# AssafSinger94/dino-tracker

Measured on NVIDIA B200. Metric: query-points/sec (854x476, T=50), higher is better.
Workload: dtype f32

## Files before the change

dino_tracker_b200/_lib.py:

```python
import ctypes
import os
from ctypes import POINTER, Structure, c_char_p, c_float, c_int, c_size_t, c_ulonglong, c_void_p

import torch

from . import build as _build

_LIB = None


class Geom(Structure):
    _fields_ = [("H", c_int), ("W", c_int), ("patch", c_int), ("stride", c_int), ("radius", c_int),
                ("h", c_int), ("w", c_int)]


class HeadWeights(Structure):
    _fields_ = [("w1", c_float * 9 * 16), ("b1", c_float * 16), ("w2", c_float * 9 * 16), ("b2", c_float)]


class Features(Structure):
    _fields_ = [("tpc", c_void_p), ("norms", c_void_p), ("hi", c_void_p), ("lo", c_void_p), ("T", c_int), ("C", c_int)]


class VitConfig(Structure):
    _fields_ = [("depth", c_int), ("dim", c_int), ("heads", c_int), ("tap_layer", c_int), ("patch", c_int), ("stride", c_int),
                ("attn_materialized", c_int), ("gemm_f16", c_int), ("gemm_pair", c_int)]


class VitWeights(Structure):
    _fields_ = [("patch_w", c_void_p), ("patch_b", c_void_p), ("cls_pos", c_void_p), ("pos", c_void_p),
                ("blocks", POINTER(c_void_p))]


class DinotrkError(RuntimeError):
    pass


_P = c_void_p
SIGNATURES = {
    "dinotrk_version": (c_int, []),
    "dinotrk_last_error": (c_char_p, []),
    "dinotrk_launch_count": (c_ulonglong, []),
    "dinotrk_make_geom": (c_int, [c_int, c_int, c_int, c_int, c_int, POINTER(Geom)]),
    "dinotrk_pack_features": (c_int, [_P, _P, _P, c_int, c_int, c_int, _P]),
    "dinotrk_unpack_features": (c_int, [_P, _P, c_int, c_int, c_int, _P]),
    "dinotrk_token_norms": (c_int, [_P, _P, c_int, c_int, c_int, _P]),
    "dinotrk_sample_descriptors": (c_int, [_P, c_int, c_int, POINTER(Geom), _P, c_int, _P, c_int, c_int, _P, _P, _P]),
    "dinotrk_split_fp16": (c_int, [_P, _P, _P, c_size_t, _P]),
    "dinotrk_corr_track_workspace_bytes": (c_size_t, [c_int, c_int, c_int, POINTER(Geom)]),
    "dinotrk_corr_track": (c_int, [POINTER(Features), POINTER(Geom), POINTER(HeadWeights), _P, _P, _P, _P, _P, _P,
                                   c_int, c_int, c_int, _P, _P, c_int, c_int, _P, c_size_t, _P]),
    "dinotrk_corr_maps_workspace_bytes": (c_size_t, [c_int, c_int, c_int]),
    "dinotrk_map_stride": (c_int, [POINTER(Geom)]),
    "dinotrk_corr_maps": (c_int, [POINTER(Features), POINTER(Geom), _P, _P, _P, _P, _P, _P, c_int, c_int, c_int,
                                  _P, _P, c_size_t, _P]),
    "dinotrk_head": (c_int, [_P, c_int, POINTER(Geom), POINTER(HeadWeights), _P, _P, c_int, c_int, _P, _P, _P]),
    "dinotrk_sample_backward": (c_int, [c_int, c_int, POINTER(Geom), _P, c_int, _P, c_int, c_int, _P, _P, _P]),
    "dinotrk_track_backward_workspace_bytes": (c_size_t, [c_int, c_int, POINTER(Geom)]),
    "dinotrk_track_backward": (c_int, [POINTER(Features), POINTER(Geom), POINTER(HeadWeights), _P, _P, c_int, _P, _P, _P, _P, _P,
                                       _P, c_int, _P, _P, _P, c_size_t, _P]),
    "dinotrk_infer_workspace_bytes": (c_size_t, [c_int, c_int, POINTER(Geom), c_int, c_int]),
    "dinotrk_infer_set_overlap": (c_int, [c_int]),
    "dinotrk_infer_set_path": (c_int, [c_int]),
    "dinotrk_infer_last_stats": (c_int, [POINTER(ctypes.c_longlong), c_int]),
    "dinotrk_infer_max_chunks": (c_size_t, [c_int, c_int, c_int]),
    "dinotrk_infer_plan": (c_int, [c_int, c_int, c_int, _P, c_int, _P, _P, c_int, _P]),
    "dinotrk_infer": (c_int, [POINTER(Features), POINTER(Geom), POINTER(HeadWeights), _P, c_int, c_float, c_float,
                              c_int, c_int, c_int, c_int, _P, _P, _P, _P, _P, c_size_t, _P]),
    "dinotrk_traj_cos_sims": (c_int, [_P, c_int, c_int, POINTER(Geom), _P, _P, c_int, _P, _P, c_size_t, _P]),
    "dinotrk_delta_workspace_bytes": (c_size_t, [c_int, c_int, c_int, POINTER(c_int)]),
    "dinotrk_delta_refine": (c_int, [_P, c_int, c_int, c_int, POINTER(c_int), POINTER(c_void_p), POINTER(c_void_p), _P,
                                     _P, _P, c_int, c_int, _P, _P, _P, c_size_t, _P]),
    "dinotrk_vit_workspace_bytes": (c_size_t, [POINTER(VitConfig), POINTER(Geom), c_int]),
    "dinotrk_vit_attention": (c_int, [_P, _P, _P, c_int, c_int, c_int, c_int, _P, _P]),
    "dinotrk_vit_forward": (c_int, [_P, c_int, POINTER(Geom), POINTER(VitConfig), POINTER(VitWeights), _P, _P, c_size_t, _P]),
    "dinotrk_best_buddies_workspace_bytes": (c_size_t, [c_int, c_int]),
    "dinotrk_best_buddies_pairs": (c_int, [POINTER(Features), POINTER(Geom), _P, _P, c_int, _P, _P, _P, c_size_t, _P]),
    "dinotrk_bb_mutual": (c_int, [_P, _P, c_int, c_int, _P, _P]),
    "dinotrk_bb_nms": (c_int, [_P, c_int, POINTER(Geom), c_float, c_float, c_int, _P, _P, _P]),
    "dinotrk_profile_classes": (c_int, []),
    "dinotrk_profile_class_name": (c_char_p, [c_int]),
    "dinotrk_profile_enable": (None, [c_int]),
    "dinotrk_profile_collect": (c_int, [POINTER(ctypes.c_double), POINTER(c_ulonglong), c_int]),
    "dinotrk_delta_refine_allgather": (c_int, [_P, c_int, c_int, c_int, POINTER(c_int), POINTER(c_void_p), POINTER(c_void_p), _P,
                                               _P, _P, c_int, c_int, _P, _P, _P, c_size_t, POINTER(c_void_p), c_int, c_size_t, _P]),
    "dinotrk_delta_refine_tc": (c_int, [_P, c_int, c_int, c_int, POINTER(c_int), POINTER(c_void_p), POINTER(c_void_p),
                                        POINTER(c_void_p), _P, _P, _P, c_int, c_int, _P, _P, _P, c_size_t, POINTER(c_void_p),
                                        c_int, c_size_t, _P]),
    "dinotrk_peer_alloc": (c_int, [c_size_t, POINTER(c_void_p), ctypes.c_char_p]),
    "dinotrk_peer_open": (c_int, [ctypes.c_char_p, POINTER(c_void_p)]),
    "dinotrk_peer_close": (c_int, [_P]),
    "dinotrk_peer_free": (c_int, [_P]),
    "dinotrk_occlusion": (c_int, [_P, _P, _P, c_int, c_int, c_float, c_float, _P, _P]),
}


def lib_path():
    return _build.LIB_PATH


def load(build_if_missing=True):
    global _LIB
    if _LIB is not None:
        return _LIB
    path = lib_path()
    if not os.path.exists(path):
        if not build_if_missing:
            raise DinotrkError(f"{path} is missing: run `python -c 'import __graft_entry__ as g; g.build()'`")
        _build.build()
    lib = ctypes.CDLL(path)
    for name, (res, args) in SIGNATURES.items():
        fn = getattr(lib, name)
        fn.restype = res
        fn.argtypes = args
    if lib.dinotrk_version() < 100:
        raise DinotrkError("libdinotrk.so is older than the Python binding")
    _LIB = lib
    return lib


def check(rc, what="dinotrk"):
    if rc != 0:
        raise DinotrkError(f"{what} failed ({rc}): {load().dinotrk_last_error().decode()}")


def ptr(t):
    if t is None:
        return None
    assert t.is_cuda and t.is_contiguous(), "device pointers must come from contiguous CUDA tensors"
    return c_void_p(t.data_ptr())


def stream_ptr(device=None):
    return c_void_p(torch.cuda.current_stream(device).cuda_stream)


def on_device(fn):
    import functools

    @functools.wraps(fn)
    def wrapped(self, *a, **kw):
        with torch.cuda.device(self._dev):
            return fn(self, *a, **kw)
    return wrapped


def require_cuda(device):
    if not torch.cuda.is_available():
        raise DinotrkError("dino_tracker_b200 needs a CUDA device (sm_100a); there is no CPU fallback")
    dev = torch.device(device)
    if dev.type != "cuda":
        raise DinotrkError(f"dino_tracker_b200 runs on CUDA only, got device={device!r}")
    return dev


def make_features(tpc, norms, hi=None, lo=None):
    f = Features()
    f.tpc, f.norms = tpc.data_ptr(), norms.data_ptr()
    f.hi = hi.data_ptr() if hi is not None else None
    f.lo = lo.data_ptr() if lo is not None else None
    f.T, f.C = tpc.shape[0], tpc.shape[2]
    f._keep = (tpc, norms, hi, lo)
    return f


def make_geom(H, W, patch=14, stride=7, radius=35):
    g = Geom()
    check(load().dinotrk_make_geom(H, W, patch, stride, radius, ctypes.byref(g)), "make_geom")
    return g


def profile_enable(on=True):
    load().dinotrk_profile_enable(1 if on else 0)


def profile_collect():
    lib = load()
    n = lib.dinotrk_profile_classes()
    ms = (ctypes.c_double * n)()
    cnt = (c_ulonglong * n)()
    check(lib.dinotrk_profile_collect(ms, cnt, n), "profile_collect")
    return {lib.dinotrk_profile_class_name(i).decode(): (ms[i], int(cnt[i])) for i in range(n) if cnt[i]}


def infer_stats():
    a = (ctypes.c_longlong * 5)()
    check(load().dinotrk_infer_last_stats(a, 5), "infer_last_stats")
    return {"anchor_maps": int(a[0]), "exact_window": int(a[1]), "full_map": int(a[2]), "pipeline": "exact-window" if a[3] else "full-map",
            "full_map_by_certificate": int(a[4])}


def launch_count():
    return int(load().dinotrk_launch_count())
```

dino_tracker_b200/csrc/inference.cu:

```cuda
#include <algorithm>
#include <vector>

#include "common.cuh"
#include "corr.cuh"
#include "sample.cuh"
#include "xwin.cuh"

namespace dtk {

constexpr int TC2_BM_ROWS = 256;

__global__ void sample_query_kernel(const float* __restrict__ tpc, int T, int C, int P, int h, int w, PointAffine pa,
                                    const float* __restrict__ qp, float* __restrict__ desc, float* __restrict__ dnorm) {
  int n = blockIdx.x;
  float x = __fadd_rn(__fmul_rn(pa.aw, qp[n * 3 + 0]), pa.bw);
  float y = __fadd_rn(__fmul_rn(pa.ah, qp[n * 3 + 1]), pa.bh);
  int tq = (int)qp[n * 3 + 2];
  tq = min(max(tq, 0), T - 1);
  TriCorners c = tri_setup(x, y, 0.f, 2, h, w);
  sample_point(tpc, C, P, c, tq, -1, desc + (size_t)n * C, dnorm + n);
}

__global__ void index_traj_kernel(const int* __restrict__ grp_frame, const int* __restrict__ grp_row0,
                                  const int* __restrict__ grp_map0, int n_groups, int n_maps, int T,
                                  int* __restrict__ out_index, float* __restrict__ traj) {
  int j = blockIdx.x * blockDim.x + threadIdx.x;
  if (j >= n_maps) return;
  int lo = 0, hi = n_groups - 1;
  while (lo < hi) {
    int mid = (lo + hi + 1) >> 1;
    if (grp_map0[mid] <= j) lo = mid; else hi = mid - 1;
  }
  int n = grp_row0[lo] + (j - grp_map0[lo]);
  int t = grp_frame[lo];
  out_index[j] = n * T + t;
  traj[((size_t)n * T + t) * 3 + 2] = (float)t;
}

__global__ void traj_cos_kernel(const float* __restrict__ tpc, int T, int C, int P, int h, int w, PointAffine pa,
                                const float* __restrict__ traj, const float* __restrict__ qp,
                                float* __restrict__ cos_out) {
  extern __shared__ __align__(16) float sm[];
  __shared__ float nrm[2];
  __shared__ float red[SAMPLE_THREADS / 32];
  const int n = blockIdx.y, i = blockIdx.x;
  int tq = (int)qp[n * 3 + 2];
  tq = min(max(tq, 0), T - 1);
  for (int which = 0; which < 2; ++which) {
    const float* pt = traj + ((size_t)n * T + (which == 0 ? tq : i)) * 3;
    float x = __fadd_rn(__fmul_rn(pa.aw, pt[0]), pa.bw);
    float y = __fadd_rn(__fmul_rn(pa.ah, pt[1]), pa.bh);
    TriCorners c = tri_setup(x, y, pt[2], T, h, w);
    sample_point(tpc, C, P, c, c.z0, c.z1, sm + which * C, nrm + which);
    __syncthreads();
  }
  const float nq = fmaxf(nrm[0], 1e-8f), ni = fmaxf(nrm[1], 1e-8f);
  float acc = 0.f;
  for (int c = threadIdx.x; c < C; c += SAMPLE_THREADS) acc = fmaf(__fdiv_rn(sm[c], nq), __fdiv_rn(sm[C + c], ni), acc);
  acc = warp_sum(acc);
  if ((threadIdx.x & 31) == 0) red[threadIdx.x >> 5] = acc;
  __syncthreads();
  if (threadIdx.x == 0) {
    float s = 0.f;
    for (int k = 0; k < SAMPLE_THREADS / 32; ++k) s += red[k];
    cos_out[(size_t)n * T + i] = s;
  }
}

__global__ void anchor_lists_kernel(const float* __restrict__ cos_sims, int N, int T, float th,
                                    int* __restrict__ cnt, int* __restrict__ qlist) {
  const int a = blockIdx.x;
  __shared__ int base;
  __shared__ int wcount[32];
  if (threadIdx.x == 0) base = 0;
  __syncthreads();
  const int lane = threadIdx.x & 31, warp = threadIdx.x >> 5, nw = blockDim.x >> 5;
  for (int n0 = 0; n0 < N; n0 += blockDim.x) {
    int n = n0 + threadIdx.x;
    bool v = n < N && cos_sims[(size_t)n * T + a] >= th;
    unsigned bal = __ballot_sync(0xffffffffu, v);
    if (lane == 0) wcount[warp] = __popc(bal);
    __syncthreads();
    int off = base;
    for (int k = 0; k < warp; ++k) off += wcount[k];
    if (v) qlist[(size_t)a * N + off + __popc(bal & ((1u << lane) - 1))] = n;
    __syncthreads();
    if (threadIdx.x == 0) {
      int tot = 0;
      for (int k = 0; k < nw; ++k) tot += wcount[k];
      base += tot;
    }
    __syncthreads();
  }
  if (threadIdx.x == 0) cnt[a] = base;
}

__global__ void sample_anchor_kernel(const float* __restrict__ tpc, int T, int C, int P, int h, int w, PointAffine pa,
                                     const float* __restrict__ traj, const int* __restrict__ qlist, int N,
                                     const int* __restrict__ grp_frame, const int* __restrict__ grp_map0,
                                     const int* __restrict__ grp_item0, int n_groups, int frame_batch,
                                     float* __restrict__ desc, float* __restrict__ dnorm, int* __restrict__ out_index,
                                     __half* __restrict__ desc_hi, __half* __restrict__ desc_lo) {
  const int j = blockIdx.x;
  int lo = 0, hi = n_groups - 1;
  while (lo < hi) {
    int mid = (lo + hi + 1) >> 1;
    if (grp_map0[mid] <= j) lo = mid; else hi = mid - 1;
  }
  const int a = grp_frame[lo];
  const int u = grp_item0[lo] + (j - grp_map0[lo]);
  const int slot = u / T, i = u - slot * T;
  const int n = qlist[(size_t)a * N + slot];
  const int i0 = (i / frame_batch) * frame_batch, e = min(i0 + frame_batch, T);
  const int Nset = e - i0 + 1;
  const float* pt = traj + ((size_t)n * T + i) * 3;
  float x = __fadd_rn(__fmul_rn(pa.aw, pt[0]), pa.bw);
  float y = __fadd_rn(__fmul_rn(pa.ah, pt[1]), pa.bh);
  TriCorners c = tri_setup(x, y, (float)(i - i0 + 1), Nset, h, w);
  int f0 = c.z0 == 0 ? a : i0 + c.z0 - 1;
  int f1 = c.z1 < 0 ? -1 : (c.z1 == 0 ? a : i0 + c.z1 - 1);
  sample_point(tpc, C, P, c, f0, f1, desc + (size_t)j * C, dnorm + j, desc_hi ? desc_hi + (size_t)j * C : nullptr,
               desc_lo ? desc_lo + (size_t)j * C : nullptr);
  if (threadIdx.x == 0) out_index[j] = (n * T + a) * T + i;
}

__global__ void sample_unique_kernel(const float* __restrict__ tpc, int T, int C, int P, int h, int w, PointAffine pa,
                                     const float* __restrict__ traj, int frame_batch, __half* __restrict__ u_hi,
                                     __half* __restrict__ u_lo, float* __restrict__ u_norm, int* __restrict__ u_flag) {
  const int u = blockIdx.x;
  const int i = u % T;
  const int i0 = (i / frame_batch) * frame_batch, e = min(i0 + frame_batch, T);
  const float* pt = traj + (size_t)u * 3;
  float x = __fadd_rn(__fmul_rn(pa.aw, pt[0]), pa.bw);
  float y = __fadd_rn(__fmul_rn(pa.ah, pt[1]), pa.bh);
  TriCorners c = tri_setup(x, y, (float)(i - i0 + 1), e - i0 + 1, h, w);
  bool slot0 = false;
#pragma unroll
  for (int k = 0; k < 4; ++k) slot0 = slot0 || (c.z0 == 0 && c.tok[k] >= 0 && c.wxy[k][0] != 0.f);
  if (threadIdx.x == 0) u_flag[u] = slot0 ? 1 : 0;
  if (slot0) return;
  const int f0 = i0 + c.z0 - 1;
  const int f1 = c.z1 < 0 ? -1 : i0 + c.z1 - 1;
  sample_point(tpc, C, P, c, f0, f1, nullptr, u_norm + u, u_hi + (size_t)u * C, u_lo + (size_t)u * C);
}

__global__ void gather_anchor_kernel(const float* __restrict__ tpc, int T, int C, int P, int h, int w, PointAffine pa,
                                     const float* __restrict__ traj, const int* __restrict__ qlist, int N,
                                     const int* __restrict__ grp_frame, const int* __restrict__ grp_map0,
                                     const int* __restrict__ grp_item0, int n_groups, int frame_batch,
                                     const __half* __restrict__ u_hi, const __half* __restrict__ u_lo,
                                     const float* __restrict__ u_norm, const int* __restrict__ u_flag,
                                     float* __restrict__ dnorm, int* __restrict__ out_index, __half* __restrict__ desc_hi,
                                     __half* __restrict__ desc_lo) {
  const int j = blockIdx.x;
  int lo = 0, hi = n_groups - 1;
  while (lo < hi) {
    int mid = (lo + hi + 1) >> 1;
    if (grp_map0[mid] <= j) lo = mid; else hi = mid - 1;
  }
  const int a = grp_frame[lo];
  const int uu = grp_item0[lo] + (j - grp_map0[lo]);
  const int slot = uu / T, i = uu - slot * T;
  const int n = qlist[(size_t)a * N + slot];
  const size_t u = (size_t)n * T + i;
  if (threadIdx.x == 0) out_index[j] = (n * T + a) * T + i;
  if (!u_flag[u]) {
    const uint4* sh = reinterpret_cast<const uint4*>(u_hi + u * C);
    const uint4* sl = reinterpret_cast<const uint4*>(u_lo + u * C);
    uint4* dh = reinterpret_cast<uint4*>(desc_hi + (size_t)j * C);
    uint4* dl = reinterpret_cast<uint4*>(desc_lo + (size_t)j * C);
    for (int k = threadIdx.x; k < C / 8; k += blockDim.x) { dh[k] = __ldg(sh + k); dl[k] = __ldg(sl + k); }
    if (threadIdx.x == 0) dnorm[j] = u_norm[u];
    return;
  }
  const int i0 = (i / frame_batch) * frame_batch, e = min(i0 + frame_batch, T);
  const float* pt = traj + u * 3;
  float x = __fadd_rn(__fmul_rn(pa.aw, pt[0]), pa.bw);
  float y = __fadd_rn(__fmul_rn(pa.ah, pt[1]), pa.bh);
  TriCorners c = tri_setup(x, y, (float)(i - i0 + 1), e - i0 + 1, h, w);
  int f0 = c.z0 == 0 ? a : i0 + c.z0 - 1;
  int f1 = c.z1 < 0 ? -1 : (c.z1 == 0 ? a : i0 + c.z1 - 1);
  sample_point(tpc, C, P, c, f0, f1, nullptr, dnorm + j, desc_hi + (size_t)j * C, desc_lo + (size_t)j * C);
}

constexpr int OCC_THREADS = 256;
__global__ void occlusion_kernel(const float* __restrict__ traj, const float* __restrict__ cos_sims,
                                 const float* __restrict__ anchors, int T, float anchor_th, float cos_th,
                                 uint8_t* __restrict__ occ) {
  extern __shared__ float sm[];
  float* med = sm;
  int* alist = reinterpret_cast<int*>(sm + T);
  float* ax = sm + 2 * T;
  float* ay = sm + 3 * T;
  const int lane = threadIdx.x & 31, warp = threadIdx.x >> 5, nw = OCC_THREADS / 32;
  float* col = sm + 4 * T + warp * T;
  __shared__ int M;
  __shared__ float th_s;
  const int n = blockIdx.x;
  if (threadIdx.x == 0) {
    int m = 0;
    for (int a = 0; a < T; ++a)
      if (cos_sims[(size_t)n * T + a] >= anchor_th) {
        alist[m] = a;
        ax[m] = traj[((size_t)n * T + a) * 3 + 0];
        ay[m] = traj[((size_t)n * T + a) * 3 + 1];
        ++m;
      }
    M = m;
  }
  __syncthreads();
  const int m = M, want = (m - 1) / 2;
  for (int i = warp; i < T; i += nw) {
    for (int p = lane; p < m; p += 32) {
      const float* g = anchors + (((size_t)n * T + alist[p]) * T + i) * 2;
      float dx = __fsub_rn(g[0], ax[p]), dy = __fsub_rn(g[1], ay[p]);
      col[p] = sqrtf(__fadd_rn(__fmul_rn(dx, dx), __fmul_rn(dy, dy)));
    }
    __syncwarp();
    for (int p = lane; p < m; p += 32) {
      const float dp = col[p];
      int rank = 0;
      for (int q = 0; q < m; ++q) {
        float dq = col[q];
        rank += (dq < dp) || (dq == dp && q < p);
      }
      if (rank == want) med[i] = dp;
    }
    __syncwarp();
  }
  __syncthreads();
  if (threadIdx.x == 0) {
    float th = -INFINITY;
    for (int p = 0; p < m; ++p) th = fmaxf(th, med[alist[p]]);
    th_s = th;
  }
  __syncthreads();
  for (int i = threadIdx.x; i < T; i += blockDim.x)
    occ[(size_t)n * T + i] = (m > 0 && (med[i] > th_s || cos_sims[(size_t)n * T + i] < cos_th)) ? 1 : 0;
}

struct GroupBuf {
  std::vector<int> v;
  int cap, n;
  explicit GroupBuf(int c) : v((size_t)5 * c), cap(c), n(0) {}
  void clear() { n = 0; }
  void push(int frame, int row0, int m, int map0, int item0) {
    v[n] = frame; v[cap + n] = row0; v[2 * cap + n] = m; v[3 * cap + n] = map0; v[4 * cap + n] = item0; ++n;
  }
};

struct ChunkMeta { int used, maxm, n_groups; bool no_thin; };
static void plan_chunks(int kind, int T, int N, const int* cnt, int ch_all, int gcap, std::vector<ChunkMeta>& metas,
                        std::vector<int>& plan_host, int align = 1, int first_cap = 0) {
  int ch = ch_all;
  metas.clear(); plan_host.clear();
  GroupBuf gb(gcap);
  auto commit_chunk = [&](int used, int maxm) {
    bool no_thin = true;
    for (int k = 0; k < gb.n; ++k) no_thin = no_thin && gb.v[2 * gb.cap + k] > STREAM_MAX_M;
    metas.push_back(ChunkMeta{used, maxm, gb.n, no_thin});
    plan_host.insert(plan_host.end(), gb.v.begin(), gb.v.end());
  };
  if (kind == 0) {
    int t = 0, row = 0;
    while (t < T) {
      gb.clear();
      int used = 0, maxm = 0;
      while (t < T && used < ch && gb.n < gcap) {
        int m = N - row;
        if (m > ch - used) m = ch - used;
        gb.push(t, row, m, used, 0);
        used += m; row += m;
        if (m > maxm) maxm = m;
        if (row == N) { row = 0; ++t; }
      }
      commit_chunk(used, maxm);
    }
  } else {
    int a = 0;
    long long item = 0;
    while (a < T) {
      gb.clear();
      int used = 0, maxm = 0;
      ch = (metas.empty() && first_cap > 0 && first_cap < ch_all) ? first_cap : ch_all;
      while (a < T && used < ch && gb.n < gcap) {
        long long tot = (long long)cnt[a] * T;
        long long m = tot - item;
        if (m > ch - used) {
          m = (long long)((ch - used) / align) * align;
          if (m == 0 && used > 0) break;
          if (m == 0) m = align;
        }
        if (m > 0) {
          gb.push(a, used, (int)m, used, (int)item);
          used += (int)m; item += m;
          if ((int)m > maxm) maxm = (int)m;
        }
        if (item >= tot) { item = 0; ++a; }
      }
      if (used == 0) break;
      commit_chunk(used, maxm);
    }
  }
}

struct CellPlan {
  std::vector<int> v;
  std::vector<size_t> first;
  std::vector<int> tiles;
  int max_m = 0;
};
static void plan_cells(int T, int gcap, const std::vector<ChunkMeta>& metas, const std::vector<int>& plan_host, CellPlan& cp) {
  const int nb = (T + XW_MAX_CELL - 1) / XW_MAX_CELL, rb = (T + nb - 1) / nb;
  cp.v.clear(); cp.first.assign(1, 0); cp.tiles.clear(); cp.max_m = 0;
  std::vector<int> r0, mm, fr, gr;
  for (size_t k = 0; k < metas.size(); ++k) {
    const int* gb = plan_host.data() + k * 5 * gcap;
    r0.clear(); mm.clear(); fr.clear(); gr.clear();
    int pre = 0;
    for (int g = 0; g < metas[k].n_groups; ++g) {
      const int frame = gb[g], row0 = gb[gcap + g], m = gb[2 * gcap + g];
      cp.tiles.push_back(pre);
      pre += (m + TC2_BM_ROWS - 1) / TC2_BM_ROWS;
      for (int s0 = 0; s0 < m; s0 += T)
        for (int b = 0; b < T; b += rb) {
          const int cm = std::min(rb, T - b);
          r0.push_back(row0 + s0 + b); mm.push_back(cm); fr.push_back(frame); gr.push_back(g);
          cp.max_m = std::max(cp.max_m, cm);
        }
    }
    for (int g = metas[k].n_groups; g <= gcap; ++g) cp.tiles.push_back(pre);
    const size_t n = r0.size();
    cp.v.insert(cp.v.end(), r0.begin(), r0.end());
    cp.v.insert(cp.v.end(), mm.begin(), mm.end());
    cp.v.insert(cp.v.end(), fr.begin(), fr.end());
    cp.v.insert(cp.v.end(), gr.begin(), gr.end());
    cp.first.push_back(cp.first.back() + n);
  }
}

struct InferAsync {
  int mode;
  cudaStream_t aux, aux2;
  cudaEvent_t fork, join, sample[2], gemm[2], head[2];
  int head_ctas_per_sm;
};
static int g_overlap_mode = -1;
struct InferAsyncSlot { InferAsync ia; int state; };
static InferAsync* infer_async() {
  static PerDev<InferAsyncSlot> slots;
  InferAsyncSlot& slot = slots.get();
  InferAsync& ia = slot.ia;
  int& state = slot.state;
  int mode = g_overlap_mode;
  if (mode < 0) {
    const char* e = getenv("DTK_OVERLAP");
    mode = e ? atoi(e) : 1;
  }
  if (mode <= 0) return nullptr;
  if (state == 0) {
    state = -1;
    const char* hc = getenv("DTK_HEAD_OVERLAP_CTAS");
    ia.head_ctas_per_sm = hc ? atoi(hc) : 2;
    if (cudaStreamCreateWithFlags(&ia.aux, cudaStreamNonBlocking) != cudaSuccess) return nullptr;
    if (cudaStreamCreateWithFlags(&ia.aux2, cudaStreamNonBlocking) != cudaSuccess) return nullptr;
    cudaEvent_t* evs[] = {&ia.fork, &ia.join, &ia.sample[0], &ia.sample[1], &ia.gemm[0], &ia.gemm[1], &ia.head[0], &ia.head[1]};
    for (cudaEvent_t* ev : evs)
      if (cudaEventCreateWithFlags(ev, cudaEventDisableTiming) != cudaSuccess) return nullptr;
    state = 1;
  }
  if (state != 1) return nullptr;
  ia.mode = mode;
  return &ia;
}

constexpr int XW_RING = 4;
constexpr int XW_PROBE_MAPS = 4096;
struct XwAsync {
  int state;
  cudaEvent_t sample[XW_RING], done[XW_RING], freed[XW_RING];
  int* host_cnt;
};
static XwAsync* xw_async() {
  static PerDev<XwAsync> slots;
  XwAsync& xa = slots.get();
  if (xa.state == 0) {
    xa.state = -1;
    for (int k = 0; k < XW_RING; ++k) {
      if (cudaEventCreateWithFlags(&xa.sample[k], cudaEventDisableTiming) != cudaSuccess) return nullptr;
      if (cudaEventCreateWithFlags(&xa.done[k], cudaEventDisableTiming) != cudaSuccess) return nullptr;
      if (cudaEventCreateWithFlags(&xa.freed[k], cudaEventDisableTiming) != cudaSuccess) return nullptr;
    }
    if (cudaHostAlloc(&xa.host_cnt, (2 * XW_RING + 16 + 4) * sizeof(int), cudaHostAllocDefault) != cudaSuccess) return nullptr;
    xa.state = 1;
  }
  return xa.state == 1 ? &xa : nullptr;
}
static int g_xw_path = -1;
static long long g_infer_stats[5] = {0, 0, 0, 0, 0};

}

using namespace dtk;

extern "C" {

int dinotrk_infer_set_path(int path) {
  DTK_CHECK_ARG(path >= -1 && path <= 1, "infer_set_path: -1 (automatic), 0 (full-map GEMM + head) or 1 (coarse pass + exact window)");
  g_xw_path = path;
  return DINOTRK_OK;
}

int dinotrk_infer_last_stats(long long* out, int n) {
  DTK_CHECK_ARG(out && n >= 4, "infer_last_stats: need at least 4 slots");
  for (int i = 0; i < (n < 5 ? n : 5); ++i) out[i] = g_infer_stats[i];
  return DINOTRK_OK;
}

static int infer_chunk_maps(int chunk_maps) { return chunk_maps > 0 ? chunk_maps : 4096; }
static int infer_chunk_eff(int chunk_maps, int T) { const int c = infer_chunk_maps(chunk_maps); return c > T ? c : T; }
static size_t infer_max_chunks(int T, int N, size_t ch) {
  size_t cap = (ch / (size_t)T) * (size_t)T;
  if (cap < (size_t)T) cap = T;
  return ((size_t)N * T * T + cap - 1) / cap + 2;
}

size_t dinotrk_infer_max_chunks(int T, int N, int chunk_maps) {
  const size_t ch = (size_t)infer_chunk_maps(chunk_maps);
  return ((size_t)N * T * T + ch - 1) / ch + 2;
}

int dinotrk_infer_plan(int kind, int T, int N, const int* anchor_counts, int chunk_maps, int* groups, int* meta,
                       int max_chunks, int* n_chunks) {
  DTK_CHECK_ARG((kind == 0 || kind == 1) && T > 0 && N >= 0 && n_chunks, "infer_plan: bad arguments");
  DTK_CHECK_ARG(kind == 0 || anchor_counts, "infer_plan: kind 1 needs the per-frame anchor counts");
  const int ch = infer_chunk_maps(chunk_maps), gcap = T + 2;
  std::vector<ChunkMeta> metas;
  std::vector<int> plan_host;
  plan_chunks(kind, T, N, anchor_counts, ch, gcap, metas, plan_host);
  *n_chunks = (int)metas.size();
  DTK_CHECK_ARG((int)metas.size() <= max_chunks || (!groups && !meta), "infer_plan: %zu chunks, room for %d", metas.size(), max_chunks);
  if (groups) std::copy(plan_host.begin(), plan_host.end(), groups);
  if (meta)
    for (size_t k = 0; k < metas.size(); ++k) {
      meta[4 * k] = metas[k].used; meta[4 * k + 1] = metas[k].maxm; meta[4 * k + 2] = metas[k].n_groups;
      meta[4 * k + 3] = metas[k].no_thin ? 1 : 0;
    }
  return DINOTRK_OK;
}

int dinotrk_infer_set_overlap(int mode) {
  DTK_CHECK_ARG(mode >= -1 && mode <= 2, "infer_set_overlap: mode must be -1 (default / DTK_OVERLAP), 0, 1 or 2");
  g_overlap_mode = mode;
  return DINOTRK_OK;
}

size_t dinotrk_corr_track_workspace_bytes(int total_maps, int n_groups, int C, const dinotrk_geom* g) {
  if (!g) return 0;
  return align_up((size_t)total_maps * dinotrk_map_stride(g) * sizeof(float), 256) + corr_plan_bytes(n_groups) +
         corr_tc_workspace_bytes(total_maps, C) + align_up((size_t)(total_maps + 1) * 4, 256) + 1024;
}

int dinotrk_corr_track(const dinotrk_features* feat, const dinotrk_geom* g,
                       const dinotrk_head_weights* hw, const float* desc, const float* desc_norm,
                       const int* grp_frame, const int* grp_row0, const int* grp_m, const int* grp_map0,
                       int n_groups, int total_maps, int max_group_m, const int* out_index, float* out,
                       int out_stride, int out_mode, void* workspace, size_t workspace_bytes, void* stream) {
  DTK_CHECK_ARG(feat && feat->tpc && feat->norms && g && hw && desc && desc_norm && grp_frame && grp_row0 && grp_m &&
                grp_map0 && out, "corr_track: null pointer");
  const int C = feat->C;
  DTK_CHECK_ARG(feat->T > 0 && C > 0 && C % 4 == 0 && n_groups >= 0 && total_maps >= 0, "corr_track: bad sizes");
  DTK_CHECK_ARG((feat->hi == nullptr) == (feat->lo == nullptr), "corr_track: hi and lo must be given together");
  DTK_CHECK_ARG(workspace && workspace_bytes >= dinotrk_corr_track_workspace_bytes(total_maps, n_groups, C, g),
                "corr_track: workspace too small");
  if (total_maps == 0) return DINOTRK_OK;
  Arena ar(workspace, workspace_bytes);
  const int ms = dinotrk_map_stride(g);
  float* maps = ar.take<float>((size_t)total_maps * ms);
  int* plan = ar.take<int>(n_groups + 1);
  float* split = ar.take<float>(corr_tc_workspace_bytes(total_maps, C) / 4);
  int* hscratch = ar.take<int>(total_maps + 1);
  cudaStream_t st = (cudaStream_t)stream;
  int rc = launch_corr_maps(make_view(*feat, *g), desc, total_maps, desc_norm, grp_frame, grp_row0, grp_m, grp_map0,
                            n_groups, total_maps, max_group_m, maps, ms, plan, split, st);
  if (rc) return rc;
  return launch_head(maps, total_maps, ms, *g, *hw, out_index, out, out_stride, out_mode, nullptr, hscratch, st);
}


size_t dinotrk_infer_workspace_bytes(int T, int C, const dinotrk_geom* g, int N, int chunk_maps) {
  if (!g) return 0;
  const size_t ch = infer_chunk_eff(chunk_maps, T), ms = dinotrk_map_stride(g);
  const int gcap = T + 2;
  size_t b = 0;
  b += align_up((size_t)N * C * 4, 256) + align_up((size_t)N * 4, 256);
  size_t c = 0;
  c += align_up(ch * ms * 4, 256);
  c += align_up(ch * C * 4, 256) + align_up(ch * 4, 256);
  c += align_up((size_t)(gcap + 1) * 4, 256);
  c += corr_tc_workspace_bytes((int)(ch > (size_t)N ? ch : (size_t)N), C) + 256;
  c += align_up((ch + 1) * 4, 256);
  c += align_up(ch * (size_t)cdiv(g->h * g->w, CORR_TILE) * 8, 256);
  b += 2 * c;
  b += 4 * align_up(ch * 4, 256);
  b += align_up(infer_max_chunks(T, N, ch) * 5 * gcap * 4, 256);
  b += align_up((size_t)T * 4, 256) + align_up((size_t)T * N * 4, 256);
  const size_t chx = ch;
  const int nb = (T + XW_MAX_CELL - 1) / XW_MAX_CELL;
  const size_t max_cells_chunk = chx + 2;
  size_t x = 0;
  x += align_up(chx * 4, 256) + corr_tc_workspace_bytes((int)chx, C) + 256 + align_up(chx * 4, 256);
  x += xw_chunk_bytes((int)chx, (int)max_cells_chunk, cdiv(g->h * g->w, XW_TILE), gcap);
  b += XW_RING * x;
  b += 2 * align_up((size_t)N * T * C * 2, 256) + 2 * align_up((size_t)N * T * 4, 256);
  b += align_up((size_t)T * g->h * g->w * 4, 256) + 256;
  b += align_up((size_t)N * T * nb * 16 + 64, 256);
  b += align_up(infer_max_chunks(T, N, ch) * (gcap + 1) * 4, 256);
  {
    const size_t sg = std::min<size_t>(infer_max_chunks(T, N, ch) * (size_t)gcap, 16384);
    b += align_up(4 * sg * 4, 256) + align_up((sg + 1) * 4, 256) + align_up(64 * 4, 256);
  }
  return b + 16384;
}

int dinotrk_traj_cos_sims(const float* tpc, int T, int C, const dinotrk_geom* g, const float* traj,
                          const float* query_points, int N, float* cos_sims, void* workspace,
                          size_t workspace_bytes, void* stream) {
  (void)workspace; (void)workspace_bytes;
  DTK_CHECK_ARG(tpc && g && traj && query_points && cos_sims, "traj_cos_sims: null pointer");
  DTK_CHECK_ARG(T > 0 && C > 0 && C % 4 == 0 && N >= 0, "traj_cos_sims: bad sizes");
  if (N == 0) return DINOTRK_OK;
  size_t smem = (size_t)2 * C * sizeof(float);
  static PerDev<size_t> attr_dev;
  size_t& attr = attr_dev.get();
  if (smem > 48 * 1024 && smem > attr) {
    DTK_CUDA(cudaFuncSetAttribute(traj_cos_kernel, cudaFuncAttributeMaxDynamicSharedMemorySize, (int)smem));
    attr = smem;
  }
  ProfRange pr(PROF_COS, (cudaStream_t)stream);
  traj_cos_kernel<<<dim3(T, N), SAMPLE_THREADS, smem, (cudaStream_t)stream>>>(
      tpc, T, C, g->h * g->w, g->h, g->w, make_point_affine(*g), traj, query_points, cos_sims);
  DTK_LAUNCHED();
  return DINOTRK_OK;
}

int dinotrk_occlusion(const float* traj, const float* cos_sims, const float* anchors, int N, int T,
                      float anchor_th, float cos_th, uint8_t* occ, void* stream) {
  DTK_CHECK_ARG(traj && cos_sims && anchors && occ && N >= 0 && T > 0, "occlusion: bad args");
  if (N == 0) return DINOTRK_OK;
  size_t smem = (size_t)(4 + OCC_THREADS / 32) * T * sizeof(float);
  DTK_CHECK_ARG(smem <= 200 * 1024, "occlusion: T=%d too large", T);
  static PerDev<size_t> attr_dev;
  size_t& attr = attr_dev.get();
  if (smem > 48 * 1024 && smem > attr) {
    DTK_CUDA(cudaFuncSetAttribute(occlusion_kernel, cudaFuncAttributeMaxDynamicSharedMemorySize, (int)smem));
    attr = smem;
  }
  ProfRange pr(PROF_OCCLUSION, (cudaStream_t)stream);
  occlusion_kernel<<<N, OCC_THREADS, smem, (cudaStream_t)stream>>>(traj, cos_sims, anchors, T, anchor_th, cos_th, occ);
  DTK_LAUNCHED();
  return DINOTRK_OK;
}

int dinotrk_infer(const dinotrk_features* feat, const dinotrk_geom* g,
                  const dinotrk_head_weights* hw, const float* query_points, int N, float anchor_th, float cos_th,
                  int frame_batch, int start_phase, int stop_after, int chunk_maps, float* traj, float* cos_sims,
                  float* anchors,
                  uint8_t* occ, void* workspace, size_t workspace_bytes, void* stream) {
  DTK_CHECK_ARG(feat && feat->tpc && feat->norms && g && hw && query_points && traj, "infer: null pointer");
  const float* tpc = feat->tpc;
  const int T = feat->T, C = feat->C;
  DTK_CHECK_ARG(T > 0 && C > 0 && C % 4 == 0 && N >= 0, "infer: bad sizes");
  DTK_CHECK_ARG((feat->hi == nullptr) == (feat->lo == nullptr), "infer: hi and lo must be given together");
  const FeatView fv = make_view(*feat, *g);
  DTK_CHECK_ARG(start_phase >= 0 && start_phase <= stop_after && stop_after <= 3,
                "infer: need 0 <= start_phase <= stop_after <= 3");
  DTK_CHECK_ARG((stop_after < 1 || cos_sims) && (stop_after < 2 || anchors) && (stop_after < 3 || occ),
                "infer: missing output buffer for the requested phases");
  DTK_CHECK_ARG(workspace && workspace_bytes >= dinotrk_infer_workspace_bytes(T, C, g, N, chunk_maps),
                "infer: workspace too small (%zu < %zu)", workspace_bytes,
                dinotrk_infer_workspace_bytes(T, C, g, N, chunk_maps));
  if (N == 0) return DINOTRK_OK;
  cudaStream_t st = (cudaStream_t)stream;
  const int P = g->h * g->w, ms = dinotrk_map_stride(g);
  const int ch = infer_chunk_eff(chunk_maps, T);
  const int fb = frame_batch > 0 ? (frame_batch < T ? frame_batch : T) : T;
  const int gcap = T + 2;
  const PointAffine pa = make_point_affine(*g);

  Arena ar(workspace, workspace_bytes);
  float* descA = ar.take<float>((size_t)N * C);
  float* normA = ar.take<float>(N);
  struct ChunkBufs {
    float* maps; float* desc; float* norm; int* plan; float* split; int* hscratch; unsigned long long* tkeys;
  } cb[2];
  int* out_index_ring[4];
  for (int k = 0; k < 2; ++k) {
    cb[k].maps = ar.take<float>((size_t)ch * ms);
    cb[k].desc = ar.take<float>((size_t)ch * C);
    cb[k].norm = ar.take<float>(ch);
    cb[k].plan = ar.take<int>(gcap + 1);
    cb[k].split = ar.take<float>(corr_tc_workspace_bytes(ch > N ? ch : N, C) / 4);
    cb[k].hscratch = ar.take<int>(ch + 1);
    cb[k].tkeys = ar.take<unsigned long long>((size_t)ch * cdiv(P, CORR_TILE));
  }
  for (int k = 0; k < 4; ++k) out_index_ring[k] = ar.take<int>(ch);
  const size_t max_chunks = infer_max_chunks(T, N, (size_t)ch);
  int* d_groups = ar.take<int>(max_chunks * 5 * gcap);
  int* d_cnt = ar.take<int>(T);
  int* d_qlist = ar.take<int>((size_t)T * N);
  struct XwSet { float* norm; float* split; int* out_index; XwChunk xc; } xr[XW_RING];
  const int n_tiles_map = cdiv(P, XW_TILE);
  __half* u_hi = ar.take<__half>((size_t)N * T * C);
  __half* u_lo = ar.take<__half>((size_t)N * T * C);
  float* u_norm = ar.take<float>((size_t)N * T);
  int* u_flag = ar.take<int>((size_t)N * T);
  float* d_rnorms = ar.take<float>((size_t)T * P);
  unsigned* d_minnorm = ar.take<unsigned>(4);
  for (int k = 0; k < XW_RING; ++k) {
    xr[k].norm = ar.take<float>(ch);
    xr[k].split = ar.take<float>(corr_tc_workspace_bytes(ch, C) / 4);
    xr[k].out_index = ar.take<int>(ch);
    XwChunk& x = xr[k].xc;
    x.key1 = ar.take<unsigned long long>((size_t)ch * n_tiles_map);
    x.max2 = ar.take<float>((size_t)ch * n_tiles_map);
    x.cand = ar.take<int>((size_t)ch * XW_MAX_CAND);
    x.stat = ar.take<int>(ch);
    x.pinfo = ar.take<int>(ch);
    x.cell_of = ar.take<int>(ch);
    x.slow_list = ar.take<int>(ch);
    x.box_org = ar.take<int2>((size_t)ch + 2);
    x.xbox = ar.take<float>((size_t)ch * XW_COLS);
    x.win = ar.take<float>((size_t)ch * 256);
    x.hin = ar.take<int2>(ch);
    x.slow_cnt = ar.take<int>(gcap + 2);
  }
  const int cell_nb = (T + XW_MAX_CELL - 1) / XW_MAX_CELL;
  int* d_cells = ar.take<int>((size_t)N * T * cell_nb * 4 + 16);
  int* d_tiles = ar.take<int>(max_chunks * (gcap + 1));
  const int sg_cap = (int)std::min<size_t>(max_chunks * (size_t)gcap, 16384);
  int* d_cgrp = ar.take<int>((size_t)4 * sg_cap);
  int* d_splan = ar.take<int>((size_t)sg_cap + 1);
  int* d_cntA = ar.take<int>(64);
  DTK_CHECK_ARG(ar.ok(), "infer: workspace arena overflow");
  const bool tensor = fv.tensor();

  std::vector<ChunkMeta> metas;
  std::vector<int> plan_host;
  auto upload_plan = [&]() -> int {
    DTK_CHECK_ARG(metas.size() <= max_chunks, "infer: chunk plan exceeds its bound (%zu > %zu)", metas.size(), max_chunks);
    if (!plan_host.empty())
      DTK_CUDA(cudaMemcpyAsync(d_groups, plan_host.data(), plan_host.size() * sizeof(int), cudaMemcpyHostToDevice, st));
    return DINOTRK_OK;
  };
  struct Grp { const int *f, *r, *m, *map0, *item; };
  auto grp_of = [&](size_t k) {
    const int* b = d_groups + k * 5 * gcap;
    return Grp{b, b + gcap, b + 2 * gcap, b + 3 * gcap, b + 4 * gcap};
  };

  int n_chunks_A = 0;
  long long maps_A = 0;
  if (start_phase <= 0) {
    NvtxRange nv("dinotrk.infer.A.trajectories");
    {
      ProfRange pr(PROF_SAMPLE, st);
      sample_query_kernel<<<N, SAMPLE_THREADS, 0, st>>>(tpc, T, C, P, g->h, g->w, pa, query_points, descA, normA);
      DTK_LAUNCHED();
    }
    if (tensor) {
      for (int k = 0; k < 2; ++k) {
        char* a_hi = reinterpret_cast<char*>(cb[k].split);
        int rc = launch_split_f16(descA, a_hi, a_hi + align_up((size_t)N * C * 2, 256), (size_t)N * C, st);
        if (rc) return rc;
      }
    }
    plan_chunks(0, T, N, nullptr, ch, gcap, metas, plan_host);
    int rc = upload_plan();
    if (rc) return rc;
    for (size_t k = 0; k < metas.size(); ++k) {
      const ChunkMeta& cm = metas[k];
      const ChunkBufs& b = cb[k & 1];
      const Grp gp = grp_of(k);
      {
        ProfRange pr(PROF_MISC, st);
        index_traj_kernel<<<cdiv(cm.used, 256), 256, 0, st>>>(gp.f, gp.r, gp.map0, cm.n_groups, cm.used, T, out_index_ring[k & 3], traj);
        DTK_LAUNCHED();
      }
      CorrAssist as;
      as.tkeys = tensor ? b.tkeys : nullptr; as.zero_word = b.hscratch; as.split_ready = tensor; as.no_thin = cm.no_thin;
      rc = launch_corr_maps(fv, descA, N, normA, gp.f, gp.r, gp.m, gp.map0, cm.n_groups, cm.used, cm.maxm, b.maps, ms, b.plan,
                            b.split, st, as);
      if (rc) return rc;
      rc = launch_head(b.maps, cm.used, ms, *g, *hw, out_index_ring[k & 3], traj, 3, 0, nullptr, b.hscratch, st, as.tkeys, true);
      if (rc) return rc;
      if (k < 16)
        DTK_CUDA(cudaMemcpyAsync(d_cntA + k, b.hscratch, sizeof(int), cudaMemcpyDeviceToDevice, st));
    }
    n_chunks_A = (int)std::min<size_t>(metas.size(), 16);
    maps_A = (long long)N * T;
  }
  if (stop_after < 1) return DINOTRK_OK;

  if (start_phase <= 1) {
    NvtxRange nv("dinotrk.infer.B.cos_sims");
    int rc = dinotrk_traj_cos_sims(tpc, T, C, g, traj, query_points, N, cos_sims, nullptr, 0, stream);
    if (rc) return rc;
  }
  if (stop_after < 2) return DINOTRK_OK;

  if (start_phase <= 2) {
    NvtxRange nv("dinotrk.infer.C.anchors");
    {
      ProfRange pr(PROF_ANCHOR_LIST, st);
      anchor_lists_kernel<<<T, 256, 0, st>>>(cos_sims, N, T, anchor_th, d_cnt, d_qlist);
      DTK_LAUNCHED();
    }
    std::vector<int> cnt(T);
    bool use_xw = tensor && g->radius <= 5 * g->stride && n_tiles_map <= 64;
    int pathsel = g_xw_path;
    if (pathsel < 0) { const char* e = getenv("DTK_XW"); if (e) pathsel = atoi(e) != 0 ? 1 : 0; }
    if (pathsel == 0) use_xw = false;
    XwAsync* xa = use_xw ? xw_async() : nullptr;
    if (!xa) use_xw = false;
    if (xa) {
      int rcn = launch_xw_rnorms(fv, d_rnorms, d_minnorm, st);
      if (rcn) return rcn;
      DTK_CUDA(cudaMemcpyAsync(xa->host_cnt + 2 * XW_RING + 16, d_minnorm, sizeof(unsigned), cudaMemcpyDeviceToHost, st));
    }
    if (xa && n_chunks_A > 0)
      DTK_CUDA(cudaMemcpyAsync(xa->host_cnt + 2 * XW_RING, d_cntA, (size_t)n_chunks_A * sizeof(int), cudaMemcpyDeviceToHost, st));
    DTK_CUDA(cudaMemcpyAsync(cnt.data(), d_cnt, (size_t)T * sizeof(int), cudaMemcpyDeviceToHost, st));
    DTK_CUDA(cudaStreamSynchronize(st));
    if (use_xw) {
      float mn;
      memcpy(&mn, xa->host_cnt + 2 * XW_RING + 16, sizeof(float));
      if (!(mn >= XW_MIN_NORM)) use_xw = false;
    }
    if (use_xw && pathsel < 0 && n_chunks_A > 0) {
      long long unc = 0;
      for (int k = 0; k < n_chunks_A; ++k) unc += xa->host_cnt[2 * XW_RING + k];
      if (unc * 4 > maps_A) use_xw = false;
    }
    long long maps_C = 0;
    for (int a = 0; a < T; ++a) maps_C += (long long)cnt[a] * T;
    g_infer_stats[0] = maps_C; g_infer_stats[1] = 0; g_infer_stats[2] = 0; g_infer_stats[3] = use_xw ? 1 : 0; g_infer_stats[4] = 0;
    size_t k0 = 0;
    bool planned = false;
    if (use_xw) {
      const bool probing = pathsel < 0;
      const int probe_cap = std::max(T, (XW_PROBE_MAPS / T) * T);
      plan_chunks(1, T, N, cnt.data(), ch, gcap, metas, plan_host, T, probing ? probe_cap : 0);
      int rc = upload_plan();
      if (rc) return rc;
      planned = true;
      CellPlan cp;
      plan_cells(T, gcap, metas, plan_host, cp);
      DTK_CHECK_ARG(cp.first.back() * 4 <= (size_t)N * T * cell_nb * 4 + 16, "infer: cell plan exceeds its bound");
      if (!cp.v.empty()) DTK_CUDA(cudaMemcpyAsync(d_cells, cp.v.data(), cp.v.size() * sizeof(int), cudaMemcpyHostToDevice, st));
      if (!cp.tiles.empty()) DTK_CUDA(cudaMemcpyAsync(d_tiles, cp.tiles.data(), cp.tiles.size() * sizeof(int), cudaMemcpyHostToDevice, st));
      InferAsync* ia = infer_async();
      const bool ovl = ia != nullptr && metas.size() > 1;
      cudaStream_t sb = ovl ? ia->aux2 : st;
      if (ovl) {
        DTK_CUDA(cudaEventRecord(ia->fork, st));
        DTK_CUDA(cudaStreamWaitEvent(sb, ia->fork, 0));
      }
      auto hi_of = [&](const XwSet& x, int rows) { (void)rows; return reinterpret_cast<char*>(x.split); };
      auto lo_of = [&](const XwSet& x, int rows) { return reinterpret_cast<char*>(x.split) + align_up((size_t)rows * C * 2, 256); };
      auto cells_of = [&](size_t k) {
        XwCells c;
        const int n = (int)(cp.first[k + 1] - cp.first[k]);
        const int* base = d_cells + 4 * cp.first[k];
        c.row0 = base; c.m = base + n; c.frame = base + 2 * n; c.group = base + 3 * n; c.n_cells = n; c.max_m = cp.max_m;
        return c;
      };
      auto enqueue_sample_x = [&](size_t k) -> int {
        const ChunkMeta& cm = metas[k];
        const XwSet& x = xr[k % XW_RING];
        const Grp gp = grp_of(k);
        if (ovl && k >= XW_RING) DTK_CUDA(cudaStreamWaitEvent(sb, xa->freed[k % XW_RING], 0));
        {
          ProfRange pr(PROF_SAMPLE, sb);
          gather_anchor_kernel<<<cm.used, SAMPLE_THREADS, 0, sb>>>(tpc, T, C, P, g->h, g->w, pa, traj, d_qlist, N, gp.f, gp.map0,
                                                                  gp.item, cm.n_groups, fb, u_hi, u_lo, u_norm, u_flag, x.norm,
                                                                  x.out_index, reinterpret_cast<__half*>(hi_of(x, cm.used)),
                                                                  reinterpret_cast<__half*>(lo_of(x, cm.used)));
          DTK_LAUNCHED();
        }
        if (ovl) DTK_CUDA(cudaEventRecord(xa->sample[k % XW_RING], sb));
        return DINOTRK_OK;
      };
      int q_rows = 0, q_groups = 0;
      auto flush = [&]() -> int {
        if (q_rows == 0) return DINOTRK_OK;
        const ChunkBufs& b = cb[0];
        CorrAssist as;
        as.tkeys = b.tkeys; as.zero_word = b.hscratch; as.split_ready = true; as.no_thin = true; as.all_wide = true; as.small_tiles = true;
        int rc2 = launch_corr_maps(fv, nullptr, ch, b.norm, d_cgrp, d_cgrp + sg_cap, d_cgrp + 2 * sg_cap, d_cgrp + 3 * sg_cap, q_groups,
                                   q_rows, q_rows, b.maps, ms, d_splan, b.split, st, as);
        if (rc2) return rc2;
        rc2 = launch_head(b.maps, q_rows, ms, *g, *hw, out_index_ring[0], anchors, 2, 0, nullptr, b.hscratch, st, b.tkeys, true);
        q_rows = q_groups = 0;
        return rc2;
      };
      auto finish = [&](size_t j) -> int {
        DTK_CUDA(cudaEventSynchronize(xa->done[j % XW_RING]));
        const int n_slow = xa->host_cnt[2 * (j % XW_RING)];
        g_infer_stats[4] += xa->host_cnt[2 * (j % XW_RING) + 1];
        const ChunkMeta& cm = metas[j];
        const XwSet& x = xr[j % XW_RING];
        const Grp gp = grp_of(j);
        DTK_CHECK_ARG(n_slow >= 0 && n_slow <= cm.used, "infer: corrupt full-map queue (%d of %d)", n_slow, cm.used);
        g_infer_stats[1] += cm.used - n_slow; g_infer_stats[2] += n_slow;
        if (n_slow > 0) {
          if (q_rows + n_slow > ch || q_groups + cm.n_groups > sg_cap) {
            int rc2 = flush();
            if (rc2) return rc2;
          }
          const ChunkBufs& b = cb[0];
          char* c_hi = reinterpret_cast<char*>(b.split);
          char* c_lo = c_hi + align_up((size_t)ch * C * 2, 256);
          int rc2 = launch_xw_compact(nullptr, hi_of(x, cm.used), lo_of(x, cm.used), x.norm, x.out_index, C, gp.f, gp.map0, cm.n_groups,
                                      n_slow, x.xc, nullptr, c_hi, c_lo, b.norm, out_index_ring[0], d_cgrp, sg_cap, st, q_rows, q_groups);
          if (rc2) return rc2;
          q_rows += n_slow; q_groups += cm.n_groups;
        }
        DTK_CUDA(cudaEventRecord(xa->freed[j % XW_RING], st));
        return DINOTRK_OK;
      };
      {
        ProfRange pr(PROF_SAMPLE, st);
        sample_unique_kernel<<<N * T, SAMPLE_THREADS, 0, st>>>(tpc, T, C, P, g->h, g->w, pa, traj, fb, u_hi, u_lo, u_norm, u_flag);
        DTK_LAUNCHED();
      }
      if (ovl) {
        DTK_CUDA(cudaEventRecord(ia->fork, st));
        DTK_CUDA(cudaStreamWaitEvent(sb, ia->fork, 0));
      }
      if (!metas.empty() && (rc = enqueue_sample_x(0))) return rc;
      size_t n_finished = 0, k_end = metas.size();
      for (size_t k = 0; k < metas.size(); ++k) {
        const ChunkMeta& cm = metas[k];
        const XwSet& x = xr[k % XW_RING];
        const Grp gp = grp_of(k);
        const XwCells cells = cells_of(k);
        if (ovl) DTK_CUDA(cudaStreamWaitEvent(st, xa->sample[k % XW_RING], 0));
        if ((rc = launch_xw_coarse(fv, hi_of(x, cm.used), cm.used, x.norm, gp.f, gp.r, gp.m, gp.map0, d_tiles + k * (gcap + 1),
                                   cm.n_groups, cm.used / TC2_BM_ROWS + cm.n_groups, x.xc, st, d_rnorms))) return rc;
        if ((rc = launch_xw_plan(cells, x.norm, cm.n_groups, *g, x.xc, st, cm.used))) return rc;
        if ((rc = launch_xw_gemm(fv, *g, hi_of(x, cm.used), lo_of(x, cm.used), cm.used, cells, x.xc, st))) return rc;
        if ((rc = launch_xw_head(fv, *g, *hw, cells, x.norm, gp.map0, cm.used, x.out_index, anchors, 2, 0, x.xc, st, cm.n_groups)))
          return rc;
        DTK_CUDA(cudaMemcpyAsync(xa->host_cnt + 2 * (k % XW_RING), x.xc.slow_cnt + cm.n_groups, 2 * sizeof(int), cudaMemcpyDeviceToHost, st));
        DTK_CUDA(cudaEventRecord(xa->done[k % XW_RING], st));
        if (k == 0 && probing && metas.size() > 1) {
          if ((rc = finish(0))) return rc;
          n_finished = 1;
          if (g_infer_stats[4] * 4 > (long long)cm.used) { k_end = 1; break; }
        }
        if (k + 1 < metas.size() && (rc = enqueue_sample_x(k + 1))) return rc;
        while (n_finished + 2 <= k)
          if ((rc = finish(n_finished++))) return rc;
      }
      while (n_finished < k_end)
        if ((rc = finish(n_finished++))) return rc;
      if ((rc = flush())) return rc;
      if (ovl) {
        DTK_CUDA(cudaEventRecord(ia->join, sb));
        DTK_CUDA(cudaStreamWaitEvent(st, ia->join, 0));
      }
      if (k_end == metas.size()) {
        if (stop_after < 3) return DINOTRK_OK;
        NvtxRange nvd("dinotrk.infer.D.occlusion");
        return dinotrk_occlusion(traj, cos_sims, anchors, N, T, anchor_th, cos_th, occ, stream);
      }
      k0 = k_end;
      g_infer_stats[3] = 0;
    }
    if (!planned) {
      plan_chunks(1, T, N, cnt.data(), ch, gcap, metas, plan_host);
      int rc0 = upload_plan();
      if (rc0) return rc0;
    }
    int rc = DINOTRK_OK;
    InferAsync* ia = infer_async();
    const bool ovl = ia != nullptr && metas.size() > k0 + 1;
    cudaStream_t sa = (ovl && ia->mode >= 2) ? ia->aux : st;
    cudaStream_t sb = ovl ? ia->aux2 : st;
    if (ovl) {
      DTK_CUDA(cudaEventRecord(ia->fork, st));
      DTK_CUDA(cudaStreamWaitEvent(sa, ia->fork, 0));
      DTK_CUDA(cudaStreamWaitEvent(sb, ia->fork, 0));
    }
    auto enqueue_sample = [&](size_t k) -> int {
      const ChunkMeta& cm = metas[k];
      const ChunkBufs& b = cb[k & 1];
      const Grp gp = grp_of(k);
      if (ovl && k >= k0 + 2) DTK_CUDA(cudaStreamWaitEvent(sb, ia->gemm[k & 1], 0));
      {
        ProfRange pr(PROF_SAMPLE, sb);
        __half* c_hi = tensor ? reinterpret_cast<__half*>(b.split) : nullptr;
        __half* c_lo = tensor ? reinterpret_cast<__half*>(reinterpret_cast<char*>(b.split) + align_up((size_t)cm.used * C * 2, 256))
                              : nullptr;
        sample_anchor_kernel<<<cm.used, SAMPLE_THREADS, 0, sb>>>(tpc, T, C, P, g->h, g->w, pa, traj, d_qlist, N, gp.f, gp.map0,
                                                                gp.item, cm.n_groups, fb, b.desc, b.norm, out_index_ring[k & 3], c_hi, c_lo);
        DTK_LAUNCHED();
      }
      if (ovl) DTK_CUDA(cudaEventRecord(ia->sample[k & 1], sb));
      return DINOTRK_OK;
    };
    auto head_full = [&](size_t j) -> int {
      const ChunkBufs& b = cb[j & 1];
      if (ovl) DTK_CUDA(cudaStreamWaitEvent(st, ia->head[j & 1], 0));
      return launch_head(b.maps, metas[j].used, ms, *g, *hw, out_index_ring[j & 3], anchors, 2, 0, nullptr, b.hscratch, st,
                         tensor ? b.tkeys : nullptr, true, 0, 2);
    };
    if (k0 < metas.size() && (rc = enqueue_sample(k0))) return rc;
    for (size_t k = k0; k < metas.size(); ++k) {
      const ChunkMeta& cm = metas[k];
      const ChunkBufs& b = cb[k & 1];
      const Grp gp = grp_of(k);
      if (ovl) DTK_CUDA(cudaStreamWaitEvent(st, ia->sample[k & 1], 0));
      if (k >= k0 + 2 && (rc = head_full(k - 2))) return rc;
      CorrAssist as;
      as.tkeys = tensor ? b.tkeys : nullptr; as.zero_word = b.hscratch; as.split_ready = tensor; as.no_thin = cm.no_thin;
      rc = launch_corr_maps(fv, b.desc, cm.used, b.norm, gp.f, gp.r, gp.m, gp.map0, cm.n_groups, cm.used, cm.maxm, b.maps, ms,
                            b.plan, b.split, st, as);
      if (rc) return rc;
      if (ovl) DTK_CUDA(cudaEventRecord(ia->gemm[k & 1], st));
      if (k + 1 < metas.size() && (rc = enqueue_sample(k + 1))) return rc;
      if (ovl) DTK_CUDA(cudaStreamWaitEvent(sa, ia->gemm[k & 1], 0));
      rc = launch_head(b.maps, cm.used, ms, *g, *hw, out_index_ring[k & 3], anchors, 2, 0, nullptr, b.hscratch, sa, as.tkeys, true,
                       (ovl && ia->mode >= 2) ? ia->head_ctas_per_sm : 0, 1);
      if (rc) return rc;
      if (ovl) DTK_CUDA(cudaEventRecord(ia->head[k & 1], sa));
    }
    for (size_t j = std::max(k0, metas.size() >= 2 ? metas.size() - 2 : 0); j < metas.size(); ++j)
      if ((rc = head_full(j))) return rc;
    if (ovl) {
      DTK_CUDA(cudaEventRecord(ia->join, sa));
      DTK_CUDA(cudaStreamWaitEvent(st, ia->join, 0));
    }
  }
  if (stop_after < 3) return DINOTRK_OK;

  NvtxRange nvd("dinotrk.infer.D.occlusion");
  return dinotrk_occlusion(traj, cos_sims, anchors, N, T, anchor_th, cos_th, occ, stream);
}

}
```

dino_tracker_b200/csrc/xwin.cu:

```cuda
#include <cuda_fp16.h>

#include "common.cuh"
#include "corr.cuh"
#include "tcgemm.cuh"
#include "tcgemm2.cuh"
#include "xwin.cuh"

namespace dtk {

int make_tmap_4d(CUtensorMap* map, const void* base, const uint64_t dims[4], const uint64_t strides_bytes[3],
                 const uint32_t box[4], int elem);

struct CoarseEpi {
  const float* rnorms;
  const float* desc_norm;
  const int* grp_frame;
  const int* grp_row0;
  const int* grp_map0;
  unsigned long long* key1;
  float* max2;
  int n_tiles, P;
  struct State { float m1[4], m2[4]; int tok[4]; };
  __device__ __forceinline__ void tile_begin(State& s) const {
#pragma unroll
    for (int a = 0; a < 4; ++a) { s.m1[a] = -INFINITY; s.m2[a] = -INFINITY; s.tok[a] = 0x7fffffff; }
  }
  __device__ __forceinline__ void tile_end(State& s, int g, int r, int nt) const {
    if (nt >= n_tiles) return;
    float m1 = s.m1[0], m2 = s.m2[0];
    int tok = s.tok[0];
#pragma unroll
    for (int a = 1; a < 4; ++a) {
      m2 = fmaxf(fmaxf(m2, s.m2[a]), fminf(m1, s.m1[a]));
      const bool take = s.m1[a] > m1 || (s.m1[a] == m1 && s.tok[a] < tok);
      tok = take ? s.tok[a] : tok;
      m1 = fmaxf(m1, s.m1[a]);
    }
    const float rdn = __fdividef(1.f, fmaxf(desc_norm[grp_row0[g] + r], XW_MIN_NORM));
    const size_t o = (size_t)(grp_map0[g] + r) * n_tiles + nt;
    key1[o] = ((unsigned long long)__float_as_uint(fmaxf(m1 * rdn, 0.f)) << 32) | (unsigned)(0x7fffffff - tok);
    max2[o] = fmaxf(m2 * rdn, 0.f);
  }
  __device__ __forceinline__ void operator()(State& s, int g, int r, int col0, const float (&f)[32], int ncols) const {
    const float* rn = rnorms + (size_t)grp_frame[g] * P + col0;
    float t[32];
#pragma unroll
    for (int i = 0; i < 32; ++i) t[i] = __ldg(rn + (i < ncols ? i : 0));
#pragma unroll
    for (int i = 0; i < 32; ++i) t[i] = i < ncols ? f[i] * t[i] : -INFINITY;
#pragma unroll
    for (int i = 0; i < 32; ++i) {
      const int a = i & 3;
      const float v = t[i];
      s.m2[a] = fmaxf(s.m2[a], fminf(s.m1[a], v));
      s.tok[a] = v > s.m1[a] ? col0 + i : s.tok[a];
      s.m1[a] = fmaxf(s.m1[a], v);
    }
  }
};

__global__ void xw_rnorm_kernel(const float* __restrict__ norms, float* __restrict__ rnorms, size_t n, unsigned* __restrict__ min_bits) {
  float mn = INFINITY;
  for (size_t i = (size_t)blockIdx.x * blockDim.x + threadIdx.x; i < n; i += (size_t)gridDim.x * blockDim.x) {
    const float v = norms[i];
    rnorms[i] = __fdiv_rn(1.f, fmaxf(v, XW_MIN_NORM));
    mn = fminf(mn, v);
  }
#pragma unroll
  for (int o = 16; o > 0; o >>= 1) mn = fminf(mn, __shfl_xor_sync(0xffffffffu, mn, o));
  if ((threadIdx.x & 31) == 0) atomicMin(min_bits, __float_as_uint(fmaxf(mn, 0.f)));
}

int launch_xw_rnorms(const FeatView& fv, float* rnorms, unsigned* min_bits, cudaStream_t st) {
  const size_t n = (size_t)fv.T * fv.P;
  DTK_CUDA(cudaMemsetAsync(min_bits, 0x7f, sizeof(unsigned), st));
  ProfRange pr(PROF_XW_PLAN, st);
  xw_rnorm_kernel<<<148 * 4, 256, 0, st>>>(fv.norms, rnorms, n, min_bits);
  DTK_LAUNCHED();
  return DINOTRK_OK;
}

int launch_xw_coarse(const FeatView& fv, const void* desc_hi, int desc_rows, const float* desc_norm, const int* grp_frame,
                     const int* grp_row0, const int* grp_m, const int* grp_map0, const int* tile_start, int n_groups,
                     int max_tiles, const XwChunk& xc, cudaStream_t st, const float* rnorms) {
  using Cfg = Tc2Cfg<TcMode::F16, 8, false>;
  using Base = TcCfg<TcMode::F16, TC2_BN>;
  static_assert(TC2_BN == 2 * XW_TILE, "coarse keys are per half GEMM tile (8 epilogue warps)");
  CUtensorMap tmA, tmB;
  int rc;
  if ((rc = make_tmap_2d(&tmA, desc_hi, desc_rows, fv.C, 128, Base::kBK, TMAP_F16))) return rc;
  if ((rc = make_tmap_3d(&tmB, fv.hi, fv.T, fv.P, fv.C, TC2_BN / 2, Base::kBK, TMAP_F16))) return rc;
  auto kern = tc_gemm2_kernel<TcMode::F16, CoarseEpi, 8>;
  static PerDev<bool> attr_dev;
  bool& attr = attr_dev.get();
  if (!attr) {
    DTK_CUDA(cudaFuncSetAttribute(kern, cudaFuncAttributeMaxDynamicSharedMemorySize, Cfg::kSmem));
    attr = true;
  }
  TcProblem pb{grp_frame, grp_row0, grp_m, tile_start, n_groups, fv.P, fv.C};
  CoarseEpi epi{rnorms, desc_norm, grp_frame, grp_row0, grp_map0, xc.key1, xc.max2, cdiv(fv.P, XW_TILE), fv.P};
  int dev = 0, sms = 148;
  cudaGetDevice(&dev);
  cudaDeviceGetAttribute(&sms, cudaDevAttrMultiProcessorCount, dev);
  const int tiles_bound = max_tiles * cdiv(fv.P, TC2_BN);
  int grid = 2 * (tiles_bound < sms / 2 ? tiles_bound : sms / 2);
  if (grid < 2) grid = 2;
  ProfRange pr(PROF_XW_COARSE, st);
  kern<<<grid, 64 + 32 * 8, Cfg::kSmem, st>>>(tmA, tmA, tmB, tmB, pb, epi);
  DTK_LAUNCHED();
  return DINOTRK_OK;
}

constexpr int PLAN_WARPS = 8;
__global__ void __launch_bounds__(PLAN_WARPS * 32)
xw_cand_kernel(int n_maps, const float* __restrict__ desc_norm, int n_groups, int n_tiles, const unsigned long long* __restrict__ key1,
               const float* __restrict__ max2, int* __restrict__ cand, int* __restrict__ pinfo, int* __restrict__ slow_cnt) {
  const int lane = threadIdx.x & 31;
  const int gw = blockIdx.x * PLAN_WARPS + (threadIdx.x >> 5), nw = gridDim.x * PLAN_WARPS;
  if (gw == 0)
    for (int i = lane; i <= n_groups + 1; i += 32) slow_cnt[i] = 0;
  for (int map = gw; map < n_maps; map += nw) {
    const unsigned long long* k1 = key1 + (size_t)map * n_tiles;
    const float* k2 = max2 + (size_t)map * n_tiles;
    unsigned long long kk[2] = {0ull, 0ull};
    float v2[2] = {0.f, 0.f};
#pragma unroll
    for (int q = 0; q < 2; ++q) {
      const int t = lane + 32 * q;
      if (t < n_tiles) { kk[q] = __ldg(k1 + t); v2[q] = __ldg(k2 + t); }
    }
    unsigned long long gk = kk[0] > kk[1] ? kk[0] : kk[1];
#pragma unroll
    for (int o = 16; o > 0; o >>= 1) { unsigned long long t = __shfl_xor_sync(0xffffffffu, gk, o); gk = t > gk ? t : gk; }
    const float gmax = __uint_as_float((unsigned)(gk >> 32));
    const int ptok = 0x7fffffff - (int)(gk & 0xffffffffu);
    const float th = gmax - 2.f * XW_EPS;
    bool amb = false;
    int ncand = 0;
#pragma unroll
    for (int q = 0; q < 2; ++q) {
      const int t = lane + 32 * q;
      const bool in = t < n_tiles;
      const bool isc = in && __uint_as_float((unsigned)(kk[q] >> 32)) >= th;
      const unsigned cm = __ballot_sync(0xffffffffu, isc);
      amb = amb || __any_sync(0xffffffffu, in && v2[q] >= th);
      const int rank = ncand + __popc(cm & ((1u << lane) - 1u));
      if (isc && rank < XW_MAX_CAND) cand[(size_t)map * XW_MAX_CAND + rank] = 0x7fffffff - (int)(kk[q] & 0xffffffffu);
      ncand += __popc(cm);
    }
    amb = amb || ncand > XW_MAX_CAND || !(gmax > 4.f * XW_EPS) || !(desc_norm[map] >= XW_MIN_NORM);
    if (lane >= ncand && lane < XW_MAX_CAND) cand[(size_t)map * XW_MAX_CAND + lane] = -1;
    if (lane == 0) pinfo[map] = amb ? -1 - ptok : ptok;
  }
}

__global__ void __launch_bounds__(PLAN_WARPS * 32)
xw_cell_kernel(XwCells cells, int w, const int* __restrict__ cand, const int* __restrict__ pinfo, int* __restrict__ stat,
               int* __restrict__ cell_of, int2* __restrict__ box_org) {
  __shared__ short s_r[PLAN_WARPS][XW_MAX_CELL], s_c[PLAN_WARPS][XW_MAX_CELL];
  __shared__ unsigned char s_ok[PLAN_WARPS][XW_MAX_CELL];
  const int lane = threadIdx.x & 31, wid = threadIdx.x >> 5;
  const int gw = blockIdx.x * PLAN_WARPS + wid, nw = gridDim.x * PLAN_WARPS;
  for (int cell = gw; cell < cells.n_cells; cell += nw) {
    const int row0 = cells.row0[cell], m = cells.m[cell];
    int nv = 0;
    for (int r = lane; r < m; r += 32) {
      const int pi = __ldg(pinfo + row0 + r);
      const int ptok = pi >= 0 ? pi : -1 - pi;
      s_r[wid][r] = (short)(ptok / w);
      s_c[wid][r] = (short)(ptok - (ptok / w) * w);
      s_ok[wid][r] = pi >= 0 ? 1 : 0;
      nv += pi >= 0 ? 1 : 0;
      cell_of[row0 + r] = cell;
    }
    __syncwarp();
#pragma unroll
    for (int o = 16; o > 0; o >>= 1) nv += __shfl_xor_sync(0xffffffffu, nv, o);
    int med_r = -1, med_c = -1;
    if (nv > 0) {
      const int want = (nv - 1) / 2;
      for (int r = lane; r < m; r += 32) {
        if (!s_ok[wid][r]) continue;
        int rk_r = 0, rk_c = 0;
        const int vr = s_r[wid][r], vc = s_c[wid][r];
        for (int q = 0; q < m; ++q) {
          if (!s_ok[wid][q]) continue;
          rk_r += (s_r[wid][q] < vr) || (s_r[wid][q] == vr && q < r);
          rk_c += (s_c[wid][q] < vc) || (s_c[wid][q] == vc && q < r);
        }
        if (rk_r == want) med_r = vr;
        if (rk_c == want) med_c = vc;
      }
#pragma unroll
      for (int o = 16; o > 0; o >>= 1) {
        med_r = max(med_r, __shfl_xor_sync(0xffffffffu, med_r, o));
        med_c = max(med_c, __shfl_xor_sync(0xffffffffu, med_c, o));
      }
    }
    int n_fit = 0;
    for (int r = lane; r < m; r += 32) {
      const int map = row0 + r;
      bool fit = s_ok[wid][r] != 0;
      if (fit) {
        const int4 cd = __ldg(reinterpret_cast<const int4*>(cand) + map);
        const int ct[4] = {cd.x, cd.y, cd.z, cd.w};
#pragma unroll
        for (int q = 0; q < XW_MAX_CAND; ++q)
          if (ct[q] >= 0) {
            const int tr = ct[q] / w, tc_ = ct[q] - tr * w;
            fit = fit && abs(tr - med_r) <= XW_SLACK && abs(tc_ - med_c) <= XW_SLACK;
          }
      }
      stat[map] = fit ? 0 : 1;
      n_fit += fit ? 1 : 0;
    }
#pragma unroll
    for (int o = 16; o > 0; o >>= 1) n_fit += __shfl_xor_sync(0xffffffffu, n_fit, o);
    if (lane == 0)
      box_org[cell] = n_fit > 0 ? make_int2(med_r - XW_BOX / 2, med_c - XW_BOX / 2) : make_int2(0, INT_MIN);
    __syncwarp();
  }
}

int launch_xw_plan(const XwCells& cells, const float* desc_norm, int n_groups, const dinotrk_geom& g, const XwChunk& xc,
                   cudaStream_t st, int n_maps) {
  static_assert(XW_MAX_CAND == 4, "candidates are read as one int4");
  const int n_tiles = cdiv(g.h * g.w, XW_TILE);
  DTK_CHECK_ARG(n_tiles <= 64, "exact-window path: token grid too large (%d tiles)", n_tiles);
  DTK_CHECK_ARG(cells.max_m <= XW_MAX_CELL, "exact-window path: cell of %d rows", cells.max_m);
  if (cells.n_cells <= 0 || n_maps <= 0) return DINOTRK_OK;
  ProfRange pr(PROF_XW_PLAN, st);
  int grid = cdiv(n_maps, PLAN_WARPS);
  if (grid > 148 * 8) grid = 148 * 8;
  xw_cand_kernel<<<grid, PLAN_WARPS * 32, 0, st>>>(n_maps, desc_norm, n_groups, n_tiles, xc.key1, xc.max2, xc.cand, xc.pinfo, xc.slow_cnt);
  DTK_LAUNCHED();
  grid = cdiv(cells.n_cells, PLAN_WARPS);
  if (grid > 148 * 8) grid = 148 * 8;
  xw_cell_kernel<<<grid, PLAN_WARPS * 32, 0, st>>>(cells, g.w, xc.cand, xc.pinfo, xc.stat, xc.cell_of, xc.box_org);
  DTK_LAUNCHED();
  return DINOTRK_OK;
}

template <int NB>
struct XwCfg {
  static constexpr int kBK = 64;
  static constexpr int kTokBytes = 128 * 128;
  static constexpr int kTokStage = 2 * kTokBytes, kTokStages = NB == 64 ? 5 : 4;
  static constexpr int kTokTx = 2 * XW_PART_TOK * 128;
  static constexpr int kLastRows = XW_BOX - (XW_PARTS - 1) * XW_PART_ROWS;
  static constexpr int kTokTxLast = 2 * kLastRows * XW_BOX * 128;
  static constexpr int kDescBytes = NB * 128;
  static constexpr int kDescStage = 2 * kDescBytes, kDescStages = 2;
  static constexpr int kSmem = kDescStages * kDescStage + kTokStages * kTokStage + 256;
  static constexpr int kAccCols = XW_PARTS * NB, kAccBufs = 512 / kAccCols;
  static constexpr uint32_t kIdesc = tc::make_idesc(0, 128, NB);
};

namespace tc {
__device__ __forceinline__ void tma_load_4d(const CUtensorMap* m, uint64_t* bar, void* dst, int c0, int c1, int c2, int c3) {
  asm volatile(
      "cp.async.bulk.tensor.4d.shared::cluster.global.mbarrier::complete_tx::bytes [%0], [%1, {%3, %4, %5, %6}], [%2];\n" ::"r"(
          smem_u32(dst)),
      "l"(m), "r"(smem_u32(bar)), "r"(c0), "r"(c1), "r"(c2), "r"(c3)
      : "memory");
}
}

template <int NB>
__global__ void __launch_bounds__(TC_THREADS, 1)
xw_gemm_kernel(const __grid_constant__ CUtensorMap tmD_hi, const __grid_constant__ CUtensorMap tmD_lo,
               const __grid_constant__ CUtensorMap tmT_hi, const __grid_constant__ CUtensorMap tmT_lo,
               const __grid_constant__ CUtensorMap tmL_hi, const __grid_constant__ CUtensorMap tmL_lo, XwCells cells,
               const int2* __restrict__ box_org, float* __restrict__ xbox, int K) {
  using Cfg = XwCfg<NB>;
  extern __shared__ uint8_t smem_raw[];
  uint8_t* smem = smem_raw;
  if (tc::smem_u32(smem) & 1023u) __trap();
  uint8_t* t_ring = smem;
  uint8_t* d_ring = smem + Cfg::kTokStages * Cfg::kTokStage;
  uint64_t* bars = reinterpret_cast<uint64_t*>(d_ring + Cfg::kDescStages * Cfg::kDescStage);
  uint64_t* d_full = bars;
  uint64_t* d_empty = d_full + Cfg::kDescStages;
  uint64_t* t_full = d_empty + Cfg::kDescStages;
  uint64_t* t_empty = t_full + Cfg::kTokStages;
  uint64_t* tfull = t_empty + Cfg::kTokStages;
  uint64_t* tempty = tfull + 2;
  uint32_t* tmem_slot = reinterpret_cast<uint32_t*>(tempty + 2);
  static_assert((2 * Cfg::kDescStages + 2 * Cfg::kTokStages + 4) * 8 + 4 <= 256, "barrier block");

  const int warp = threadIdx.x >> 5, lane = threadIdx.x & 31;
  const int KB = (K + Cfg::kBK - 1) / Cfg::kBK;

  if (warp == 0 && lane == 0) {
    tc::prefetch_tmap(&tmD_hi); tc::prefetch_tmap(&tmD_lo); tc::prefetch_tmap(&tmT_hi); tc::prefetch_tmap(&tmT_lo);
    tc::prefetch_tmap(&tmL_hi); tc::prefetch_tmap(&tmL_lo);
    for (int s = 0; s < Cfg::kDescStages; ++s) { tc::mbar_init(&d_full[s], 1); tc::mbar_init(&d_empty[s], 1); }
    for (int s = 0; s < Cfg::kTokStages; ++s) { tc::mbar_init(&t_full[s], 1); tc::mbar_init(&t_empty[s], 1); }
    for (int s = 0; s < 2; ++s) { tc::mbar_init(&tfull[s], 1); tc::mbar_init(&tempty[s], 4); }
    tc::mbar_fence_init();
  }
  if (warp == 1) tc::tmem_alloc(tmem_slot, 512);
  tc::fence_before_sync();
  __syncthreads();
  tc::fence_after_sync();
  const uint32_t tmem_base = *tmem_slot;

  if (warp == 0) {
    if (tc::elect_one()) {
      int ds = 0, dph = 0, ts = 0, tph = 0;
      for (int cell = blockIdx.x; cell < cells.n_cells; cell += gridDim.x) {
        const int2 org = box_org[cell];
        if (org.y == INT_MIN) continue;
        const int drow = cells.row0[cell], frame = cells.frame[cell];
        for (int kb = 0; kb < KB; ++kb) {
          const int k0 = kb * Cfg::kBK;
          tc::mbar_wait(&d_empty[ds], dph ^ 1);
          uint8_t* sd = d_ring + ds * Cfg::kDescStage;
          tc::mbar_expect_tx(&d_full[ds], Cfg::kDescStage);
          tc::tma_load_2d(&tmD_hi, &d_full[ds], sd, k0, drow);
          tc::tma_load_2d(&tmD_lo, &d_full[ds], sd + Cfg::kDescBytes, k0, drow);
          if (++ds == Cfg::kDescStages) { ds = 0; dph ^= 1; }
          for (int part = 0; part < XW_PARTS; ++part) {
            tc::mbar_wait(&t_empty[ts], tph ^ 1);
            uint8_t* st = t_ring + ts * Cfg::kTokStage;
            if (part < XW_PARTS - 1) {
              tc::mbar_expect_tx(&t_full[ts], Cfg::kTokTx);
              tc::tma_load_4d(&tmT_hi, &t_full[ts], st, k0, org.y, org.x + part * XW_PART_ROWS, frame);
              tc::tma_load_4d(&tmT_lo, &t_full[ts], st + Cfg::kTokBytes, k0, org.y, org.x + part * XW_PART_ROWS, frame);
            } else {
              tc::mbar_expect_tx(&t_full[ts], Cfg::kTokTxLast);
              tc::tma_load_4d(&tmL_hi, &t_full[ts], st, k0, org.y, org.x + part * XW_PART_ROWS, frame);
              tc::tma_load_4d(&tmL_lo, &t_full[ts], st + Cfg::kTokBytes, k0, org.y, org.x + part * XW_PART_ROWS, frame);
            }
            if (++ts == Cfg::kTokStages) { ts = 0; tph ^= 1; }
          }
        }
      }
    }
  } else if (warp == 1) {
    int ds = 0, dph = 0, ts = 0, tph = 0, it = 0;
    for (int cell = blockIdx.x; cell < cells.n_cells; cell += gridDim.x) {
      if (box_org[cell].y == INT_MIN) continue;
      const int buf = it % Cfg::kAccBufs, use = it / Cfg::kAccBufs;
      tc::mbar_wait(&tempty[buf], (use & 1) ^ 1);
      tc::fence_after_sync();
      for (int kb = 0; kb < KB; ++kb) {
        tc::mbar_wait(&d_full[ds], dph);
        const uint32_t sd = tc::smem_u32(d_ring + ds * Cfg::kDescStage);
        for (int part = 0; part < XW_PARTS; ++part) {
          tc::mbar_wait(&t_full[ts], tph);
          tc::fence_after_sync();
          if (tc::elect_one()) {
            const uint32_t st = tc::smem_u32(t_ring + ts * Cfg::kTokStage);
            const uint32_t tmem_d = tmem_base + buf * Cfg::kAccCols + part * NB;
#pragma unroll
            for (int ks = 0; ks < Cfg::kBK / 16; ++ks) {
              const uint32_t koff = ks * 32;
              const uint64_t t_hi = tc::smem_desc_sw128(st + koff), t_lo = tc::smem_desc_sw128(st + Cfg::kTokBytes + koff);
              const uint64_t d_hi = tc::smem_desc_sw128(sd + koff), d_lo = tc::smem_desc_sw128(sd + Cfg::kDescBytes + koff);
              const uint32_t first = (kb == 0 && ks == 0) ? 0u : 1u;
              tc::mma_ss<false>(tmem_d, t_hi, d_lo, Cfg::kIdesc, first);
              tc::mma_ss<false>(tmem_d, t_lo, d_hi, Cfg::kIdesc, 1u);
              tc::mma_ss<false>(tmem_d, t_hi, d_hi, Cfg::kIdesc, 1u);
            }
            tc::mma_commit(&t_empty[ts]);
            if (part == XW_PARTS - 1) {
              tc::mma_commit(&d_empty[ds]);
              if (kb == KB - 1) tc::mma_commit(&tfull[buf]);
            }
          }
          __syncwarp();
          if (++ts == Cfg::kTokStages) { ts = 0; tph ^= 1; }
        }
        if (++ds == Cfg::kDescStages) { ds = 0; dph ^= 1; }
      }
      ++it;
    }
  } else {
    const int quad = warp & 3;
    int it = 0;
    for (int cell = blockIdx.x; cell < cells.n_cells; cell += gridDim.x) {
      if (box_org[cell].y == INT_MIN) continue;
      const int m = cells.m[cell], map0 = cells.row0[cell];
      const int buf = it % Cfg::kAccBufs, use = it / Cfg::kAccBufs;
      tc::mbar_wait(&tfull[buf], use & 1);
      tc::fence_after_sync();
      const int tok = quad * 32 + lane;
#pragma unroll 1
      for (int part = 0; part < XW_PARTS; ++part) {
        const int col = part * XW_PART_TOK + tok;
        const bool ok = tok < XW_PART_TOK && col < XW_BOX * XW_BOX;
        const uint32_t taddr = tmem_base + ((uint32_t)(quad * 32) << 16) + buf * Cfg::kAccCols + part * NB;
        float* dst = xbox + (size_t)map0 * XW_COLS + col;
#pragma unroll 1
        for (int c = 0; c < NB && c < m; c += 32) {
          uint32_t v[32];
          tc::tmem_ld32(taddr + c, v);
          tc::tmem_ld_wait();
          if (ok) {
#pragma unroll
            for (int i = 0; i < 32; ++i)
              if (c + i < m) dst[(size_t)(c + i) * XW_COLS] = __uint_as_float(v[i]);
          }
        }
      }
      tc::fence_before_sync();
      __syncwarp();
      if (lane == 0) tc::mbar_arrive(&tempty[buf]);
      ++it;
    }
  }

  tc::fence_before_sync();
  __syncthreads();
  if (warp == 1) {
    tc::fence_after_sync();
    tc::tmem_dealloc(tmem_base, 512);
  }
}

int launch_xw_gemm(const FeatView& fv, const dinotrk_geom& g, const void* desc_hi, const void* desc_lo, int desc_rows,
                   const XwCells& cells, const XwChunk& xc, cudaStream_t st) {
  if (cells.n_cells <= 0) return DINOTRK_OK;
  DTK_CHECK_ARG(fv.C % 8 == 0 && cells.max_m <= XW_MAX_CELL, "exact-window GEMM: bad sizes");
  const bool small = cells.max_m <= 64;
  const int nb = small ? 64 : 128;
  CUtensorMap tD_hi, tD_lo, tT_hi, tT_lo, tL_hi, tL_lo;
  int rc;
  if ((rc = make_tmap_2d(&tD_hi, desc_hi, desc_rows, fv.C, nb, 64, TMAP_F16))) return rc;
  if ((rc = make_tmap_2d(&tD_lo, desc_lo, desc_rows, fv.C, nb, 64, TMAP_F16))) return rc;
  const uint64_t dims[4] = {(uint64_t)fv.C, (uint64_t)g.w, (uint64_t)g.h, (uint64_t)fv.T};
  const uint64_t strides[3] = {(uint64_t)fv.C * 2, (uint64_t)g.w * fv.C * 2, (uint64_t)fv.P * fv.C * 2};
  const uint32_t box[4] = {64, XW_BOX, XW_PART_ROWS, 1};
  if ((rc = make_tmap_4d(&tT_hi, fv.hi, dims, strides, box, TMAP_F16))) return rc;
  if ((rc = make_tmap_4d(&tT_lo, fv.lo, dims, strides, box, TMAP_F16))) return rc;
  const uint32_t box_last[4] = {64, XW_BOX, (uint32_t)XwCfg<64>::kLastRows, 1};
  if ((rc = make_tmap_4d(&tL_hi, fv.hi, dims, strides, box_last, TMAP_F16))) return rc;
  if ((rc = make_tmap_4d(&tL_lo, fv.lo, dims, strides, box_last, TMAP_F16))) return rc;
  static PerDev<bool> attr_dev;
  bool& attr = attr_dev.get();
  if (!attr) {
    DTK_CUDA(cudaFuncSetAttribute(xw_gemm_kernel<64>, cudaFuncAttributeMaxDynamicSharedMemorySize, XwCfg<64>::kSmem));
    DTK_CUDA(cudaFuncSetAttribute(xw_gemm_kernel<128>, cudaFuncAttributeMaxDynamicSharedMemorySize, XwCfg<128>::kSmem));
    attr = true;
  }
  int dev = 0, sms = 148;
  cudaGetDevice(&dev);
  cudaDeviceGetAttribute(&sms, cudaDevAttrMultiProcessorCount, dev);
  const int grid = cells.n_cells < sms ? cells.n_cells : sms;
  ProfRange pr(PROF_XW_GEMM, st);
  if (small)
    xw_gemm_kernel<64><<<grid, TC_THREADS, XwCfg<64>::kSmem, st>>>(tD_hi, tD_lo, tT_hi, tT_lo, tL_hi, tL_lo, cells, xc.box_org, xc.xbox, fv.C);
  else
    xw_gemm_kernel<128><<<grid, TC_THREADS, XwCfg<128>::kSmem, st>>>(tD_hi, tD_lo, tT_hi, tT_lo, tL_hi, tL_lo, cells, xc.box_org, xc.xbox, fv.C);
  DTK_LAUNCHED();
  return DINOTRK_OK;
}

constexpr int XH_WARPS = 8;
constexpr int XH_MP = 18;
constexpr int XWM = 15, XWH = 13, XWB = 11;
constexpr int XH_MWIN = 544;
constexpr int XH_PER_WARP = XH_MWIN + XWH * XWH * 16;
constexpr int XH_WTAB = 20 * 16;
constexpr int XH_SMEM = (XH_WTAB + XH_WARPS * XH_PER_WARP) * 4;

struct XhParams {
  int h, w, P, n_tiles;
  int stride_px, half_patch, radius2;
  float normW, normH;
  int out_stride, out_mode;
  float P1[16], P2[16];
};

template <bool INTERIOR>
__device__ __forceinline__ void xw_refine(const XhParams& hp, const float2* __restrict__ wtab, float b2w, float2* __restrict__ mm2,
                                          float2* __restrict__ hh2, const float (&wv)[8], int arow, int acol, int lane,
                                          float& zmax, float (&tot)[5]) {
  const int h = hp.h, w = hp.w;
  const int cp = lane & 7, pg = lane >> 3;
#pragma unroll
  for (int q = 0; q < 8; ++q) {
    const int i = lane + 32 * q;
    const int y = i >> 4, x = i & 15;
    if (y < XWM && x < XWM) mm2[y * XH_MP + x] = make_float2(wv[q], wv[q]);
  }
  __syncwarp();
  {
    float2 w1r[9];
#pragma unroll
    for (int k = 0; k < 9; ++k) w1r[k] = wtab[k * 8 + cp];
    const float2 b1r = wtab[9 * 8 + cp];
    for (int y = pg; y < XWH; y += 4) {
      const int r = arow - 6 + y;
      const bool row_in = r >= 0 && r < h;
      const float2* m0 = mm2 + y * XH_MP;
      float2 in0[16], in1[16], in2[16];
#pragma unroll
      for (int x = 0; x < 16; x += 2) {
        const float4 q0 = *reinterpret_cast<const float4*>(m0 + x);
        const float4 q1 = *reinterpret_cast<const float4*>(m0 + XH_MP + x);
        const float4 q2 = *reinterpret_cast<const float4*>(m0 + 2 * XH_MP + x);
        in0[x] = make_float2(q0.x, q0.y); in0[x + 1] = make_float2(q0.z, q0.w);
        in1[x] = make_float2(q1.x, q1.y); in1[x + 1] = make_float2(q1.z, q1.w);
        in2[x] = make_float2(q2.x, q2.y); in2[x + 1] = make_float2(q2.z, q2.w);
      }
#pragma unroll
      for (int x = 0; x < XWH; ++x) {
        float2 a0 = __ffma2_rn(w1r[0], in0[x], b1r), a1 = __fmul2_rn(w1r[3], in1[x]), a2 = __fmul2_rn(w1r[6], in2[x]);
        a0 = __ffma2_rn(w1r[1], in0[x + 1], a0); a1 = __ffma2_rn(w1r[4], in1[x + 1], a1); a2 = __ffma2_rn(w1r[7], in2[x + 1], a2);
        a0 = __ffma2_rn(w1r[2], in0[x + 2], a0); a1 = __ffma2_rn(w1r[5], in1[x + 2], a1); a2 = __ffma2_rn(w1r[8], in2[x + 2], a2);
        const float2 a = __fadd2_rn(__fadd2_rn(a0, a1), a2);
        const int c = acol - 6 + x;
        const bool in = INTERIOR || (row_in && c >= 0 && c < w);
        hh2[(y * XWH + x) * 8 + cp] = in ? make_float2(fmaxf(a.x, 0.f), fmaxf(a.y, 0.f)) : make_float2(0.f, 0.f);
      }
    }
  }
  __syncwarp();
  float* zb = reinterpret_cast<float*>(mm2);
  {
    float2 w2r[9];
#pragma unroll
    for (int k = 0; k < 9; ++k) w2r[k] = wtab[(10 + k) * 8 + cp];
#pragma unroll
    for (int yi = 0; yi < 3; ++yi) {
      const int y = pg + 4 * yi;
      const bool row_ok = y < XWB;
      const float2* h0 = hh2 + ((row_ok ? y : 0) * XWH) * 8 + cp;
      float2 i00 = h0[0], i01 = h0[8], i10 = h0[XWH * 8], i11 = h0[(XWH + 1) * 8];
      float2 i20 = h0[2 * XWH * 8], i21 = h0[(2 * XWH + 1) * 8];
      float v[12];
      v[11] = 0.f;
#pragma unroll
      for (int x = 0; x < XWB; ++x) {
        const float2 i02 = h0[(x + 2) * 8], i12 = h0[(XWH + x + 2) * 8], i22 = h0[(2 * XWH + x + 2) * 8];
        float2 a0 = __fmul2_rn(w2r[0], i00), a1 = __fmul2_rn(w2r[3], i10), a2 = __fmul2_rn(w2r[6], i20);
        a0 = __ffma2_rn(w2r[1], i01, a0); a1 = __ffma2_rn(w2r[4], i11, a1); a2 = __ffma2_rn(w2r[7], i21, a2);
        a0 = __ffma2_rn(w2r[2], i02, a0); a1 = __ffma2_rn(w2r[5], i12, a1); a2 = __ffma2_rn(w2r[8], i22, a2);
        const float2 a = __fadd2_rn(__fadd2_rn(a0, a1), a2);
        v[x] = a.x + a.y;
        i00 = i01; i01 = i02; i10 = i11; i11 = i12; i20 = i21; i21 = i22;
      }
      const bool b2 = cp & 4, b1 = cp & 2, b0 = cp & 1;
      float u[6], w3[3];
#pragma unroll
      for (int j = 0; j < 6; ++j) {
        const float send = b2 ? v[j] : v[j + 6], keep = b2 ? v[j + 6] : v[j];
        u[j] = keep + __shfl_xor_sync(0xffffffffu, send, 4);
      }
#pragma unroll
      for (int j = 0; j < 3; ++j) {
        const float send = b1 ? u[j] : u[j + 3], keep = b1 ? u[j + 3] : u[j];
        w3[j] = keep + __shfl_xor_sync(0xffffffffu, send, 2);
      }
      const float t0 = (b0 ? w3[2] : w3[0]) + __shfl_xor_sync(0xffffffffu, b0 ? w3[0] : w3[2], 1);
      const float t1 = (b0 ? 0.f : w3[1]) + __shfl_xor_sync(0xffffffffu, b0 ? w3[1] : 0.f, 1);
      const int idx0 = (b2 ? 6 : 0) + (b1 ? 3 : 0) + (b0 ? 2 : 0);
      if (row_ok && idx0 < XWB) zb[y * XWB + idx0] = t0 + b2w;
      if (row_ok && !b0) zb[y * XWB + idx0 + 1] = t1 + b2w;
    }
  }
  __syncwarp();
  float z[4];
  bool valid[4], indisc[4];
  float px[4], py[4];
  zmax = -INFINITY;
#pragma unroll
  for (int q = 0; q < 4; ++q) {
    const int p = lane + 32 * q;
    valid[q] = false; indisc[q] = false; z[q] = -INFINITY; px[q] = py[q] = 0.f;
    if (p < XWB * XWB) {
      const int y = p / XWB, x = p - y * XWB;
      const int r = arow - 5 + y, c = acol - 5 + x;
      valid[q] = INTERIOR || (r >= 0 && r < h && c >= 0 && c < w);
      if (valid[q]) {
        z[q] = zb[p];
        const int dr = (r - arow) * hp.stride_px, dc = (c - acol) * hp.stride_px;
        indisc[q] = dr * dr + dc * dc <= hp.radius2;
        px[q] = (float)(hp.half_patch + c * hp.stride_px);
        py[q] = (float)(hp.half_patch + r * hp.stride_px);
      }
    }
    zmax = fmaxf(zmax, z[q]);
  }
  zmax = warp_max(zmax);
#pragma unroll
  for (int q = 0; q < 4; ++q) {
    const float e = valid[q] ? expf(z[q] - zmax) : 0.f;
    tot[0] += e;
    if (indisc[q]) { tot[1] += e; tot[2] = fmaf(px[q], e, tot[2]); tot[3] = fmaf(py[q], e, tot[3]); }
    tot[4] += valid[q] ? 1.f : 0.f;
  }
}

constexpr int XWIN_PITCH = 256;
__global__ void __launch_bounds__(256)
xw_window_kernel(int n_maps, int h, int w, int P, int n_tiles, const float* __restrict__ norms, const float* __restrict__ desc_norm,
                 const int* __restrict__ cell_frame, const int* __restrict__ cell_of, const int2* __restrict__ box_org,
                 const int* __restrict__ stat, const int* __restrict__ cand, const unsigned long long* __restrict__ key1,
                 const float* __restrict__ max2, const float* __restrict__ xbox, float* __restrict__ win, int2* __restrict__ hin) {
  const int lane = threadIdx.x & 31;
  const int gw = (blockIdx.x * blockDim.x + threadIdx.x) >> 5, nw = (gridDim.x * blockDim.x) >> 5;
  for (int map = gw; map < n_maps; map += nw) {
    if (stat[map] != 0) {
      if (lane == 0) hin[map] = make_int2(-1, 0);
      continue;
    }
    const int cell = cell_of[map];
    const int2 org = box_org[cell];
    const float* fn = norms + (size_t)cell_frame[cell] * P;
    const float* xr = xbox + (size_t)map * XW_COLS;
    const float dn = desc_norm[map];
    const int4 cd = __ldg(reinterpret_cast<const int4*>(cand) + map);
    const int ct[4] = {cd.x, cd.y, cd.z, cd.w};
    float best = -1.f;
    int amax = -1;
#pragma unroll
    for (int q = 0; q < XW_MAX_CAND; ++q)
      if (ct[q] >= 0) {
        const int tr = ct[q] / w, tcn = ct[q] - tr * w;
        const float v = fmaxf(__fdiv_rn(__ldg(xr + xw_col(tr - org.x, tcn - org.y)), fmaxf(__fmul_rn(dn, __ldg(fn + ct[q])), 1e-8f)), 0.f);
        if (v > best || (v == best && ct[q] < amax)) { best = v; amax = ct[q]; }
      }
    const int arow = amax / w, acol = amax - arow * w;
    float mout = 0.f;
    for (int t = lane; t < n_tiles; t += 32) {
      const unsigned long long k = __ldg(key1 + (size_t)map * n_tiles + t);
      const int tk = 0x7fffffff - (int)(k & 0xffffffffu);
      const int tr = tk / w, tcn = tk - tr * w;
      const bool in_core = abs(tr - arow) <= 3 && abs(tcn - acol) <= 3;
      const float b = in_core ? __ldg(max2 + (size_t)map * n_tiles + t) : __uint_as_float((unsigned)(k >> 32));
      mout = fmaxf(mout, b + XW_EPS);
    }
#pragma unroll
    for (int q = 0; q < 8; ++q) {
      const int i = lane + 32 * q;
      const int y = i >> 4, x = i & 15;
      const int r = arow - 7 + y, c = acol - 7 + x;
      float v = 0.f;
      if (y < XWM && x < XWM && r >= 0 && r < h && c >= 0 && c < w) {
        v = fmaxf(__fdiv_rn(__ldg(xr + xw_col(r - org.x, c - org.y)), fmaxf(__fmul_rn(dn, __ldg(fn + r * w + c)), 1e-8f)), 0.f);
        if (!(abs(r - arow) <= 3 && abs(c - acol) <= 3)) mout = fmaxf(mout, v);
      }
      win[(size_t)map * XWIN_PITCH + i] = v;
    }
    mout = warp_max(mout);
    if (lane == 0) hin[map] = make_int2(amax, __float_as_int(mout));
  }
}

__global__ void __launch_bounds__(XH_WARPS * 32, 2)
xw_head_kernel(int n_maps, XhParams hp, dinotrk_head_weights wts, const int* __restrict__ cell_group, const int* __restrict__ grp_map0,
               const int* __restrict__ cell_of, const float* __restrict__ win, const int2* __restrict__ hin,
               const int* __restrict__ out_index, float* __restrict__ out, int* __restrict__ slow_cnt, int* __restrict__ slow_list,
               int n_groups) {
  extern __shared__ __align__(16) float xh_smem[];
  const int lane = threadIdx.x & 31, wid = __shfl_sync(0xffffffffu, (int)(threadIdx.x >> 5), 0);
  float2* wtab = reinterpret_cast<float2*>(xh_smem);
  float2* mm = reinterpret_cast<float2*>(xh_smem + XH_WTAB + wid * XH_PER_WARP);
  float2* hh_ = reinterpret_cast<float2*>(xh_smem + XH_WTAB + wid * XH_PER_WARP + XH_MWIN);
  if (threadIdx.x < 19 * 8) {
    const int k = threadIdx.x >> 3, c = threadIdx.x & 7;
    wtab[threadIdx.x] = k < 9    ? make_float2(wts.w1[c][k], wts.w1[c + 8][k])
                        : k == 9 ? make_float2(wts.b1[c], wts.b1[c + 8])
                                 : make_float2(wts.w2[c][k - 10], wts.w2[c + 8][k - 10]);
  }
  __syncthreads();
  const int h = hp.h, w = hp.w, P = hp.P;
  const int stride = gridDim.x * XH_WARPS;

  int map = blockIdx.x * XH_WARPS + wid;
  float wnext[8];
  int2 hnext = make_int2(-1, 0);
  if (map < n_maps) {
    hnext = __ldg(hin + map);
#pragma unroll
    for (int q = 0; q < 8; ++q) wnext[q] = __ldg(win + (size_t)map * XWIN_PITCH + lane + 32 * q);
  }
  for (; map < n_maps; map += stride) {
    float wv[8];
#pragma unroll
    for (int q = 0; q < 8; ++q) wv[q] = wnext[q];
    const int2 hcur = hnext;
    if (map + stride < n_maps) {
      hnext = __ldg(hin + map + stride);
#pragma unroll
      for (int q = 0; q < 8; ++q) wnext[q] = __ldg(win + (size_t)(map + stride) * XWIN_PITCH + lane + 32 * q);
    }
    const bool slow = hcur.x < 0;
    const int amax = hcur.x;
    const float mout = __int_as_float(hcur.y);
    float zmax = 0.f;
    float tot[5] = {0.f, 0.f, 0.f, 0.f, 0.f};
    if (!slow) {
      const int arow = amax / w, acol = amax - arow * w;
      if (arow >= 7 && arow + 7 < h && acol >= 7 && acol + 7 < w)
        xw_refine<true>(hp, wtab, wts.b2, mm, hh_, wv, arow, acol, lane, zmax, tot);
      else
        xw_refine<false>(hp, wtab, wts.b2, mm, hh_, wv, arow, acol, lane, zmax, tot);
#pragma unroll
      for (int q = 0; q < 5; ++q) tot[q] = warp_sum(tot[q]);
    }
    if (lane == 0) {
      bool certified = false;
      if (!slow) {
        float F = wts.b2;
#pragma unroll
        for (int o = 0; o < 16; ++o) F = fmaf(hp.P2[o], fmaxf(fmaf(hp.P1[o], mout, wts.b1[o]), 0.f), F);
        const float rest = ((float)P - tot[4]) * expf(fminf(F - zmax, 80.f));
        certified = tot[1] >= 2e-8f * (tot[0] + rest) && tot[1] > 0.f && isfinite(rest);
      }
      if (certified) {
        const float px_ = __fdiv_rn(tot[2], tot[1]), py_ = __fdiv_rn(tot[3], tot[1]);
        float nx = __fadd_rn(__fmul_rn(2.f, __fdiv_rn(px_, hp.normW)), -1.f);
        float ny = __fadd_rn(__fmul_rn(2.f, __fdiv_rn(py_, hp.normH)), -1.f);
        if (hp.out_mode == 0) {
          nx = __fmul_rn(__fdiv_rn(__fadd_rn(nx, 1.f), 2.f), hp.normW);
          ny = __fmul_rn(__fdiv_rn(__fadd_rn(ny, 1.f), 2.f), hp.normH);
        }
        const size_t oi = (size_t)(out_index ? out_index[map] : map) * hp.out_stride;
        out[oi] = nx; out[oi + 1] = ny;
      } else {
        const int g = cell_group[cell_of[map]];
        const int pos = atomicAdd(slow_cnt + g, 1);
        slow_list[grp_map0[g] + pos] = map;
        atomicAdd(slow_cnt + n_groups, 1);
        if (!slow) atomicAdd(slow_cnt + n_groups + 1, 1);
      }
    }
    __syncwarp();
  }
}

int launch_xw_head(const FeatView& fv, const dinotrk_geom& g, const dinotrk_head_weights& hw, const XwCells& cells,
                   const float* desc_norm, const int* grp_map0, int n_maps, const int* out_index, float* out, int out_stride,
                   int out_mode, const XwChunk& xc, cudaStream_t st, int n_groups) {
  if (n_maps <= 0) return DINOTRK_OK;
  DTK_CHECK_ARG(g.radius <= 5 * g.stride, "exact-window path: disc radius %d exceeds 5 tokens", g.radius);
  XhParams hp;
  hp.h = g.h; hp.w = g.w; hp.P = g.h * g.w; hp.n_tiles = cdiv(hp.P, XW_TILE);
  hp.stride_px = g.stride; hp.half_patch = g.patch / 2; hp.radius2 = g.radius * g.radius;
  hp.normW = (float)(g.W - 1); hp.normH = (float)(g.H - 1);
  hp.out_stride = out_stride; hp.out_mode = out_mode;
  for (int o = 0; o < 16; ++o) {
    float p1 = 0.f, p2 = 0.f;
    for (int k = 0; k < 9; ++k) { p1 += hw.w1[o][k] > 0.f ? hw.w1[o][k] : 0.f; p2 += hw.w2[o][k] > 0.f ? hw.w2[o][k] : 0.f; }
    hp.P1[o] = p1 * (1.f + 1e-6f); hp.P2[o] = p2 * (1.f + 1e-6f);
  }
  int dev = 0, sms = 148;
  cudaGetDevice(&dev);
  cudaDeviceGetAttribute(&sms, cudaDevAttrMultiProcessorCount, dev);
  int grid = cdiv(n_maps, XH_WARPS);
  if (grid > sms * 2) grid = sms * 2;
  static PerDev<bool> attr_dev;
  bool& attr = attr_dev.get();
  if (!attr) {
    DTK_CUDA(cudaFuncSetAttribute(xw_head_kernel, cudaFuncAttributeMaxDynamicSharedMemorySize, XH_SMEM));
    attr = true;
  }
  ProfRange pr(PROF_XW_HEAD, st);
  {
    int wgrid = cdiv(n_maps, 8);
    if (wgrid > sms * 8) wgrid = sms * 8;
    xw_window_kernel<<<wgrid, 256, 0, st>>>(n_maps, g.h, g.w, hp.P, hp.n_tiles, fv.norms, desc_norm, cells.frame, xc.cell_of, xc.box_org,
                                            xc.stat, xc.cand, xc.key1, xc.max2, xc.xbox, xc.win, xc.hin);
    DTK_LAUNCHED();
  }
  xw_head_kernel<<<grid, XH_WARPS * 32, XH_SMEM, st>>>(n_maps, hp, hw, cells.group, grp_map0, xc.cell_of, xc.win, xc.hin, out_index,
                                                 out, xc.slow_cnt, xc.slow_list, n_groups);
  DTK_LAUNCHED();
  return DINOTRK_OK;
}

__global__ void __launch_bounds__(128)
xw_compact_kernel(const float4* __restrict__ desc, const uint4* __restrict__ dhi, const uint4* __restrict__ dlo,
                  const float* __restrict__ desc_norm, const int* __restrict__ out_index, int C, const int* __restrict__ grp_frame,
                  const int* __restrict__ grp_map0, int n_groups, const int* __restrict__ slow_cnt,
                  const int* __restrict__ slow_list, float4* __restrict__ c_desc, uint4* __restrict__ c_hi, uint4* __restrict__ c_lo,
                  float* __restrict__ c_norm, int* __restrict__ c_out_index, int* __restrict__ cgrp, int gcap, int row_base,
                  int grp_base) {
  __shared__ int s_g, s_pos;
  const int bb = blockIdx.x;
  if (threadIdx.x == 0) {
    int pre = 0, gsel = -1, psel = 0;
    for (int g = 0; g < n_groups; ++g) {
      const int c = slow_cnt[g];
      if (bb == 0) {
        cgrp[grp_base + g] = grp_frame[g]; cgrp[gcap + grp_base + g] = row_base + pre; cgrp[2 * gcap + grp_base + g] = c;
        cgrp[3 * gcap + grp_base + g] = row_base + pre;
      }
      if (gsel < 0 && bb < pre + c) { gsel = g; psel = bb - pre; }
      pre += c;
    }
    s_g = gsel; s_pos = psel;
  }
  __syncthreads();
  if (s_g < 0) return;
  const int b = row_base + bb;
  const int src = slow_list[grp_map0[s_g] + s_pos];
  if (desc != nullptr)
    for (int i = threadIdx.x; i < C / 4; i += blockDim.x) c_desc[(size_t)b * (C / 4) + i] = desc[(size_t)src * (C / 4) + i];
  if (dhi != nullptr)
    for (int i = threadIdx.x; i < C / 8; i += blockDim.x) {
      c_hi[(size_t)b * (C / 8) + i] = dhi[(size_t)src * (C / 8) + i];
      c_lo[(size_t)b * (C / 8) + i] = dlo[(size_t)src * (C / 8) + i];
    }
  if (threadIdx.x == 0) { c_norm[b] = desc_norm[src]; c_out_index[b] = out_index[src]; }
}

int launch_xw_compact(const float* desc, const void* desc_hi, const void* desc_lo, const float* desc_norm,
                      const int* out_index, int C, const int* grp_frame, const int* grp_map0, int n_groups, int n_slow,
                      const XwChunk& xc, float* c_desc, void* c_hi, void* c_lo, float* c_norm, int* c_out_index, int* cgrp,
                      int gcap, cudaStream_t st, int row_base, int grp_base) {
  if (n_slow <= 0) return DINOTRK_OK;
  ProfRange pr(PROF_MISC, st);
  xw_compact_kernel<<<n_slow, 128, 0, st>>>(reinterpret_cast<const float4*>(desc), reinterpret_cast<const uint4*>(desc_hi),
                                            reinterpret_cast<const uint4*>(desc_lo), desc_norm, out_index, C, grp_frame, grp_map0,
                                            n_groups, xc.slow_cnt, xc.slow_list, reinterpret_cast<float4*>(c_desc),
                                            reinterpret_cast<uint4*>(c_hi), reinterpret_cast<uint4*>(c_lo), c_norm, c_out_index, cgrp,
                                            gcap, row_base, grp_base);
  DTK_LAUNCHED();
  return DINOTRK_OK;
}

size_t xw_chunk_bytes(int chunk_maps, int max_cells, int n_tiles, int gcap) {
  const size_t ch = (size_t)chunk_maps;
  size_t b = 0;
  b += align_up(ch * n_tiles * 8, 256) + align_up(ch * n_tiles * 4, 256);
  b += align_up(ch * XW_MAX_CAND * 4, 256) + 4 * align_up(ch * 4, 256);
  b += align_up((size_t)max_cells * 8, 256);
  b += align_up(ch * XW_COLS * 4, 256);
  b += align_up(ch * 256 * 4, 256) + align_up(ch * 8, 256);
  b += align_up((size_t)(gcap + 2) * 4, 256);
  return b + 2048;
}

}
```

dino_tracker_b200/csrc/xwin.cuh:

```cuda
#pragma once
#include "common.cuh"
#include "corr.cuh"

namespace dtk {

constexpr float XW_EPS = 1.1e-3f;
constexpr int XW_BOX = 21;
constexpr int XW_SLACK = 3;
constexpr int XW_PARTS = 4, XW_PART_ROWS = 6;
constexpr int XW_PART_TOK = XW_PART_ROWS * XW_BOX;
constexpr int XW_COLS = 448;
constexpr int XW_MAX_CELL = 128;
constexpr int XW_MAX_CAND = 4;
constexpr float XW_MIN_NORM = 1e-4f;
constexpr int XW_TILE = 128;

__host__ __device__ inline int xw_col(int by, int bx) { return by * XW_BOX + bx; }

struct XwChunk {
  unsigned long long* key1;
  float* max2;
  int* cand;
  int* pinfo;
  int* stat;
  int* cell_of;
  int2* box_org;
  float* xbox;
  float* win;
  int2* hin;
  int* slow_cnt;
  int* slow_list;
};

struct XwCells {
  const int* row0;
  const int* m;
  const int* frame;
  const int* group;
  int n_cells, max_m;
};

size_t xw_chunk_bytes(int chunk_maps, int max_cells, int n_tiles, int gcap);
int launch_xw_coarse(const FeatView& fv, const void* desc_hi, int desc_rows, const float* desc_norm, const int* grp_frame,
                     const int* grp_row0, const int* grp_m, const int* grp_map0, const int* tile_start, int n_groups,
                     int max_tiles, const XwChunk& xc, cudaStream_t st, const float* rnorms);
int launch_xw_rnorms(const FeatView& fv, float* rnorms, unsigned* min_bits, cudaStream_t st);
int launch_xw_plan(const XwCells& cells, const float* desc_norm, int n_groups, const dinotrk_geom& g, const XwChunk& xc,
                   cudaStream_t st, int n_maps);
int launch_xw_gemm(const FeatView& fv, const dinotrk_geom& g, const void* desc_hi, const void* desc_lo, int desc_rows,
                   const XwCells& cells, const XwChunk& xc, cudaStream_t st);
int launch_xw_head(const FeatView& fv, const dinotrk_geom& g, const dinotrk_head_weights& hw, const XwCells& cells,
                   const float* desc_norm, const int* grp_map0, int n_maps, const int* out_index, float* out, int out_stride,
                   int out_mode, const XwChunk& xc, cudaStream_t st, int n_groups);
int launch_xw_compact(const float* desc, const void* desc_hi, const void* desc_lo, const float* desc_norm,
                      const int* out_index, int C, const int* grp_frame, const int* grp_map0, int n_groups, int n_slow,
                      const XwChunk& xc, float* c_desc, void* c_hi, void* c_lo, float* c_norm, int* c_out_index, int* cgrp,
                      int gcap, cudaStream_t st, int row_base = 0, int grp_base = 0);

}
```

Baseline: 13300.

## Size exact-window GEMM boxes to the candidate spread per cell

Each cell's token box is now sized from the actual min/max of its fitting candidate rows and columns instead of a fixed 21x21 box in four parts. Narrow cells (span at most 16 columns) use a 16-wide tensor-map box with 8-row parts, and short cells issue fewer M-parts. The intent is fewer TMA loads and fewer tcgemm MMAs per cell. It adds a per-cell box struct, a second tensor-map pair, and per-part-count statistics, with a variable row stride in the xbox indexing.

Result: faster. 14160 (median of 6 runs) (+6.5%).

```diff
diff --git a/dino_tracker_b200/_lib.py b/dino_tracker_b200/_lib.py
--- a/dino_tracker_b200/_lib.py
+++ b/dino_tracker_b200/_lib.py
@@ -184,10 +184,10 @@
 
 
 def infer_stats():
-    a = (ctypes.c_longlong * 5)()
-    check(load().dinotrk_infer_last_stats(a, 5), "infer_last_stats")
+    a = (ctypes.c_longlong * 8)()
+    check(load().dinotrk_infer_last_stats(a, 8), "infer_last_stats")
     return {"anchor_maps": int(a[0]), "exact_window": int(a[1]), "full_map": int(a[2]), "pipeline": "exact-window" if a[3] else "full-map",
-            "full_map_by_certificate": int(a[4])}
+            "full_map_by_certificate": int(a[4]), "exact_window_cells_by_parts": {p: int(a[3 + p]) for p in (2, 3, 4)}}
 
 
 def launch_count():
diff --git a/dino_tracker_b200/csrc/inference.cu b/dino_tracker_b200/csrc/inference.cu
--- a/dino_tracker_b200/csrc/inference.cu
+++ b/dino_tracker_b200/csrc/inference.cu
@@ -391,13 +391,14 @@
       if (cudaEventCreateWithFlags(&xa.done[k], cudaEventDisableTiming) != cudaSuccess) return nullptr;
       if (cudaEventCreateWithFlags(&xa.freed[k], cudaEventDisableTiming) != cudaSuccess) return nullptr;
     }
-    if (cudaHostAlloc(&xa.host_cnt, (2 * XW_RING + 16 + 4) * sizeof(int), cudaHostAllocDefault) != cudaSuccess) return nullptr;
+    if (cudaHostAlloc(&xa.host_cnt, (XW_NCNT * XW_RING + 16 + 4) * sizeof(int), cudaHostAllocDefault) != cudaSuccess) return nullptr;
     xa.state = 1;
   }
   return xa.state == 1 ? &xa : nullptr;
 }
 static int g_xw_path = -1;
-static long long g_infer_stats[5] = {0, 0, 0, 0, 0};
+constexpr int INFER_NSTATS = 5 + (XW_PARTS - 1);
+static long long g_infer_stats[INFER_NSTATS] = {};
 
 }
 
@@ -413,7 +414,7 @@
 
 int dinotrk_infer_last_stats(long long* out, int n) {
   DTK_CHECK_ARG(out && n >= 4, "infer_last_stats: need at least 4 slots");
-  for (int i = 0; i < (n < 5 ? n : 5); ++i) out[i] = g_infer_stats[i];
+  for (int i = 0; i < (n < INFER_NSTATS ? n : INFER_NSTATS); ++i) out[i] = g_infer_stats[i];
   return DINOTRK_OK;
 }
 
@@ -629,11 +630,11 @@
     x.pinfo = ar.take<int>(ch);
     x.cell_of = ar.take<int>(ch);
     x.slow_list = ar.take<int>(ch);
-    x.box_org = ar.take<int2>((size_t)ch + 2);
+    x.box = ar.take<XwBox>((size_t)ch + 2);
     x.xbox = ar.take<float>((size_t)ch * XW_COLS);
     x.win = ar.take<float>((size_t)ch * 256);
     x.hin = ar.take<int2>(ch);
-    x.slow_cnt = ar.take<int>(gcap + 2);
+    x.slow_cnt = ar.take<int>(gcap + XW_NCNT);
   }
   const int cell_nb = (T + XW_MAX_CELL - 1) / XW_MAX_CELL;
   int* d_cells = ar.take<int>((size_t)N * T * cell_nb * 4 + 16);
@@ -726,25 +727,26 @@
     if (xa) {
       int rcn = launch_xw_rnorms(fv, d_rnorms, d_minnorm, st);
       if (rcn) return rcn;
-      DTK_CUDA(cudaMemcpyAsync(xa->host_cnt + 2 * XW_RING + 16, d_minnorm, sizeof(unsigned), cudaMemcpyDeviceToHost, st));
+      DTK_CUDA(cudaMemcpyAsync(xa->host_cnt + XW_NCNT * XW_RING + 16, d_minnorm, sizeof(unsigned), cudaMemcpyDeviceToHost, st));
     }
     if (xa && n_chunks_A > 0)
-      DTK_CUDA(cudaMemcpyAsync(xa->host_cnt + 2 * XW_RING, d_cntA, (size_t)n_chunks_A * sizeof(int), cudaMemcpyDeviceToHost, st));
+      DTK_CUDA(cudaMemcpyAsync(xa->host_cnt + XW_NCNT * XW_RING, d_cntA, (size_t)n_chunks_A * sizeof(int), cudaMemcpyDeviceToHost, st));
     DTK_CUDA(cudaMemcpyAsync(cnt.data(), d_cnt, (size_t)T * sizeof(int), cudaMemcpyDeviceToHost, st));
     DTK_CUDA(cudaStreamSynchronize(st));
     if (use_xw) {
       float mn;
-      memcpy(&mn, xa->host_cnt + 2 * XW_RING + 16, sizeof(float));
+      memcpy(&mn, xa->host_cnt + XW_NCNT * XW_RING + 16, sizeof(float));
       if (!(mn >= XW_MIN_NORM)) use_xw = false;
     }
     if (use_xw && pathsel < 0 && n_chunks_A > 0) {
       long long unc = 0;
-      for (int k = 0; k < n_chunks_A; ++k) unc += xa->host_cnt[2 * XW_RING + k];
+      for (int k = 0; k < n_chunks_A; ++k) unc += xa->host_cnt[XW_NCNT * XW_RING + k];
       if (unc * 4 > maps_A) use_xw = false;
     }
     long long maps_C = 0;
     for (int a = 0; a < T; ++a) maps_C += (long long)cnt[a] * T;
-    g_infer_stats[0] = maps_C; g_infer_stats[1] = 0; g_infer_stats[2] = 0; g_infer_stats[3] = use_xw ? 1 : 0; g_infer_stats[4] = 0;
+    for (long long& v : g_infer_stats) v = 0;
+    g_infer_stats[0] = maps_C; g_infer_stats[3] = use_xw ? 1 : 0;
     size_t k0 = 0;
     bool planned = false;
     if (use_xw) {
@@ -806,8 +808,9 @@
       };
       auto finish = [&](size_t j) -> int {
         DTK_CUDA(cudaEventSynchronize(xa->done[j % XW_RING]));
-        const int n_slow = xa->host_cnt[2 * (j % XW_RING)];
-        g_infer_stats[4] += xa->host_cnt[2 * (j % XW_RING) + 1];
+        const int* hc = xa->host_cnt + XW_NCNT * (j % XW_RING);
+        const int n_slow = hc[0];
+        for (int i = 1; i < XW_NCNT; ++i) g_infer_stats[3 + i] += hc[i];
         const ChunkMeta& cm = metas[j];
         const XwSet& x = xr[j % XW_RING];
         const Grp gp = grp_of(j);
@@ -852,7 +855,8 @@
         if ((rc = launch_xw_gemm(fv, *g, hi_of(x, cm.used), lo_of(x, cm.used), cm.used, cells, x.xc, st))) return rc;
         if ((rc = launch_xw_head(fv, *g, *hw, cells, x.norm, gp.map0, cm.used, x.out_index, anchors, 2, 0, x.xc, st, cm.n_groups)))
           return rc;
-        DTK_CUDA(cudaMemcpyAsync(xa->host_cnt + 2 * (k % XW_RING), x.xc.slow_cnt + cm.n_groups, 2 * sizeof(int), cudaMemcpyDeviceToHost, st));
+        DTK_CUDA(cudaMemcpyAsync(xa->host_cnt + XW_NCNT * (k % XW_RING), x.xc.slow_cnt + cm.n_groups, XW_NCNT * sizeof(int),
+                                 cudaMemcpyDeviceToHost, st));
         DTK_CUDA(cudaEventRecord(xa->done[k % XW_RING], st));
         if (k == 0 && probing && metas.size() > 1) {
           if ((rc = finish(0))) return rc;
diff --git a/dino_tracker_b200/csrc/xwin.cu b/dino_tracker_b200/csrc/xwin.cu
--- a/dino_tracker_b200/csrc/xwin.cu
+++ b/dino_tracker_b200/csrc/xwin.cu
@@ -118,7 +118,7 @@
   const int lane = threadIdx.x & 31;
   const int gw = blockIdx.x * PLAN_WARPS + (threadIdx.x >> 5), nw = gridDim.x * PLAN_WARPS;
   if (gw == 0)
-    for (int i = lane; i <= n_groups + 1; i += 32) slow_cnt[i] = 0;
+    for (int i = lane; i < n_groups + XW_NCNT; i += 32) slow_cnt[i] = 0;
   for (int map = gw; map < n_maps; map += nw) {
     const unsigned long long* k1 = key1 + (size_t)map * n_tiles;
     const float* k2 = max2 + (size_t)map * n_tiles;
@@ -156,7 +156,7 @@
 
 __global__ void __launch_bounds__(PLAN_WARPS * 32)
 xw_cell_kernel(XwCells cells, int w, const int* __restrict__ cand, const int* __restrict__ pinfo, int* __restrict__ stat,
-               int* __restrict__ cell_of, int2* __restrict__ box_org) {
+               int* __restrict__ cell_of, XwBox* __restrict__ box, int* __restrict__ part_cnt) {
   __shared__ short s_r[PLAN_WARPS][XW_MAX_CELL], s_c[PLAN_WARPS][XW_MAX_CELL];
   __shared__ unsigned char s_ok[PLAN_WARPS][XW_MAX_CELL];
   const int lane = threadIdx.x & 31, wid = threadIdx.x >> 5;
@@ -197,10 +197,11 @@
         med_c = max(med_c, __shfl_xor_sync(0xffffffffu, med_c, o));
       }
     }
-    int n_fit = 0;
+    int n_fit = 0, r_lo = INT_MAX, r_hi = INT_MIN, c_lo = INT_MAX, c_hi = INT_MIN;
     for (int r = lane; r < m; r += 32) {
       const int map = row0 + r;
       bool fit = s_ok[wid][r] != 0;
+      int mr_lo = INT_MAX, mr_hi = INT_MIN, mc_lo = INT_MAX, mc_hi = INT_MIN;
       if (fit) {
         const int4 cd = __ldg(reinterpret_cast<const int4*>(cand) + map);
         const int ct[4] = {cd.x, cd.y, cd.z, cd.w};
@@ -209,15 +210,30 @@
           if (ct[q] >= 0) {
             const int tr = ct[q] / w, tc_ = ct[q] - tr * w;
             fit = fit && abs(tr - med_r) <= XW_SLACK && abs(tc_ - med_c) <= XW_SLACK;
+            mr_lo = min(mr_lo, tr); mr_hi = max(mr_hi, tr); mc_lo = min(mc_lo, tc_); mc_hi = max(mc_hi, tc_);
           }
       }
       stat[map] = fit ? 0 : 1;
       n_fit += fit ? 1 : 0;
-    }
-#pragma unroll
-    for (int o = 16; o > 0; o >>= 1) n_fit += __shfl_xor_sync(0xffffffffu, n_fit, o);
-    if (lane == 0)
-      box_org[cell] = n_fit > 0 ? make_int2(med_r - XW_BOX / 2, med_c - XW_BOX / 2) : make_int2(0, INT_MIN);
+      if (fit) { r_lo = min(r_lo, mr_lo); r_hi = max(r_hi, mr_hi); c_lo = min(c_lo, mc_lo); c_hi = max(c_hi, mc_hi); }
+    }
+#pragma unroll
+    for (int o = 16; o > 0; o >>= 1) {
+      n_fit += __shfl_xor_sync(0xffffffffu, n_fit, o);
+      r_lo = min(r_lo, __shfl_xor_sync(0xffffffffu, r_lo, o)); r_hi = max(r_hi, __shfl_xor_sync(0xffffffffu, r_hi, o));
+      c_lo = min(c_lo, __shfl_xor_sync(0xffffffffu, c_lo, o)); c_hi = max(c_hi, __shfl_xor_sync(0xffffffffu, c_hi, o));
+    }
+    if (lane == 0) {
+      XwBox b{0, 0, 0, 0, 0};
+      if (n_fit > 0) {
+        const int height = r_hi - r_lo + 15;
+        const bool wide = c_hi - c_lo + 15 > XW_NARROW;
+        const int rows = wide ? XW_ROWS_WIDE : XW_ROWS_NARROW;
+        b = XwBox{r_lo - 7, c_lo - 7, (short)(wide ? XW_BOX : XW_NARROW), (short)height, (short)((height + rows - 1) / rows)};
+        atomicAdd(part_cnt + b.parts - 2, 1);
+      }
+      box[cell] = b;
+    }
     __syncwarp();
   }
 }
@@ -236,7 +252,8 @@
   DTK_LAUNCHED();
   grid = cdiv(cells.n_cells, PLAN_WARPS);
   if (grid > 148 * 8) grid = 148 * 8;
-  xw_cell_kernel<<<grid, PLAN_WARPS * 32, 0, st>>>(cells, g.w, xc.cand, xc.pinfo, xc.stat, xc.cell_of, xc.box_org);
+  xw_cell_kernel<<<grid, PLAN_WARPS * 32, 0, st>>>(cells, g.w, xc.cand, xc.pinfo, xc.stat, xc.cell_of, xc.box,
+                                                   xc.slow_cnt + n_groups + 2);
   DTK_LAUNCHED();
   return DINOTRK_OK;
 }
@@ -246,9 +263,8 @@
   static constexpr int kBK = 64;
   static constexpr int kTokBytes = 128 * 128;
   static constexpr int kTokStage = 2 * kTokBytes, kTokStages = NB == 64 ? 5 : 4;
-  static constexpr int kTokTx = 2 * XW_PART_TOK * 128;
-  static constexpr int kLastRows = XW_BOX - (XW_PARTS - 1) * XW_PART_ROWS;
-  static constexpr int kTokTxLast = 2 * kLastRows * XW_BOX * 128;
+  static constexpr int kTokTxNarrow = 2 * XW_ROWS_NARROW * XW_NARROW * 128, kTokTxWide = 2 * XW_ROWS_WIDE * XW_BOX * 128;
+  static_assert(XW_ROWS_NARROW * XW_NARROW <= 128 && XW_ROWS_WIDE * XW_BOX <= 128, "an M-part is at most 128 tokens");
   static constexpr int kDescBytes = NB * 128;
   static constexpr int kDescStage = 2 * kDescBytes, kDescStages = 2;
   static constexpr int kSmem = kDescStages * kDescStage + kTokStages * kTokStage + 256;
@@ -269,9 +285,9 @@
 template <int NB>
 __global__ void __launch_bounds__(TC_THREADS, 1)
 xw_gemm_kernel(const __grid_constant__ CUtensorMap tmD_hi, const __grid_constant__ CUtensorMap tmD_lo,
-               const __grid_constant__ CUtensorMap tmT_hi, const __grid_constant__ CUtensorMap tmT_lo,
-               const __grid_constant__ CUtensorMap tmL_hi, const __grid_constant__ CUtensorMap tmL_lo, XwCells cells,
-               const int2* __restrict__ box_org, float* __restrict__ xbox, int K) {
+               const __grid_constant__ CUtensorMap tmN_hi, const __grid_constant__ CUtensorMap tmN_lo,
+               const __grid_constant__ CUtensorMap tmW_hi, const __grid_constant__ CUtensorMap tmW_lo, XwCells cells,
+               const XwBox* __restrict__ box, float* __restrict__ xbox, int K) {
   using Cfg = XwCfg<NB>;
   extern __shared__ uint8_t smem_raw[];
   uint8_t* smem = smem_raw;
@@ -292,8 +308,8 @@
   const int KB = (K + Cfg::kBK - 1) / Cfg::kBK;
 
   if (warp == 0 && lane == 0) {
-    tc::prefetch_tmap(&tmD_hi); tc::prefetch_tmap(&tmD_lo); tc::prefetch_tmap(&tmT_hi); tc::prefetch_tmap(&tmT_lo);
-    tc::prefetch_tmap(&tmL_hi); tc::prefetch_tmap(&tmL_lo);
+    tc::prefetch_tmap(&tmD_hi); tc::prefetch_tmap(&tmD_lo); tc::prefetch_tmap(&tmN_hi); tc::prefetch_tmap(&tmN_lo);
+    tc::prefetch_tmap(&tmW_hi); tc::prefetch_tmap(&tmW_lo);
     for (int s = 0; s < Cfg::kDescStages; ++s) { tc::mbar_init(&d_full[s], 1); tc::mbar_init(&d_empty[s], 1); }
     for (int s = 0; s < Cfg::kTokStages; ++s) { tc::mbar_init(&t_full[s], 1); tc::mbar_init(&t_empty[s], 1); }
     for (int s = 0; s < 2; ++s) { tc::mbar_init(&tfull[s], 1); tc::mbar_init(&tempty[s], 4); }
@@ -309,8 +325,12 @@
     if (tc::elect_one()) {
       int ds = 0, dph = 0, ts = 0, tph = 0;
       for (int cell = blockIdx.x; cell < cells.n_cells; cell += gridDim.x) {
-        const int2 org = box_org[cell];
-        if (org.y == INT_MIN) continue;
+        const XwBox bx = box[cell];
+        if (bx.parts == 0) continue;
+        const bool wide = bx.width == XW_BOX;
+        const CUtensorMap* tm_hi = wide ? &tmW_hi : &tmN_hi;
+        const CUtensorMap* tm_lo = wide ? &tmW_lo : &tmN_lo;
+        const int rows = wide ? XW_ROWS_WIDE : XW_ROWS_NARROW, tx = wide ? Cfg::kTokTxWide : Cfg::kTokTxNarrow;
         const int drow = cells.row0[cell], frame = cells.frame[cell];
         for (int kb = 0; kb < KB; ++kb) {
           const int k0 = kb * Cfg::kBK;
@@ -320,18 +340,12 @@
           tc::tma_load_2d(&tmD_hi, &d_full[ds], sd, k0, drow);
           tc::tma_load_2d(&tmD_lo, &d_full[ds], sd + Cfg::kDescBytes, k0, drow);
           if (++ds == Cfg::kDescStages) { ds = 0; dph ^= 1; }
-          for (int part = 0; part < XW_PARTS; ++part) {
+          for (int part = 0; part < bx.parts; ++part) {
             tc::mbar_wait(&t_empty[ts], tph ^ 1);
             uint8_t* st = t_ring + ts * Cfg::kTokStage;
-            if (part < XW_PARTS - 1) {
-              tc::mbar_expect_tx(&t_full[ts], Cfg::kTokTx);
-              tc::tma_load_4d(&tmT_hi, &t_full[ts], st, k0, org.y, org.x + part * XW_PART_ROWS, frame);
-              tc::tma_load_4d(&tmT_lo, &t_full[ts], st + Cfg::kTokBytes, k0, org.y, org.x + part * XW_PART_ROWS, frame);
-            } else {
-              tc::mbar_expect_tx(&t_full[ts], Cfg::kTokTxLast);
-              tc::tma_load_4d(&tmL_hi, &t_full[ts], st, k0, org.y, org.x + part * XW_PART_ROWS, frame);
-              tc::tma_load_4d(&tmL_lo, &t_full[ts], st + Cfg::kTokBytes, k0, org.y, org.x + part * XW_PART_ROWS, frame);
-            }
+            tc::mbar_expect_tx(&t_full[ts], tx);
+            tc::tma_load_4d(tm_hi, &t_full[ts], st, k0, bx.col, bx.row + part * rows, frame);
+            tc::tma_load_4d(tm_lo, &t_full[ts], st + Cfg::kTokBytes, k0, bx.col, bx.row + part * rows, frame);
             if (++ts == Cfg::kTokStages) { ts = 0; tph ^= 1; }
           }
         }
@@ -340,14 +354,15 @@
   } else if (warp == 1) {
     int ds = 0, dph = 0, ts = 0, tph = 0, it = 0;
     for (int cell = blockIdx.x; cell < cells.n_cells; cell += gridDim.x) {
-      if (box_org[cell].y == INT_MIN) continue;
+      const int parts = box[cell].parts;
+      if (parts == 0) continue;
       const int buf = it % Cfg::kAccBufs, use = it / Cfg::kAccBufs;
       tc::mbar_wait(&tempty[buf], (use & 1) ^ 1);
       tc::fence_after_sync();
       for (int kb = 0; kb < KB; ++kb) {
         tc::mbar_wait(&d_full[ds], dph);
         const uint32_t sd = tc::smem_u32(d_ring + ds * Cfg::kDescStage);
-        for (int part = 0; part < XW_PARTS; ++part) {
+        for (int part = 0; part < parts; ++part) {
           tc::mbar_wait(&t_full[ts], tph);
           tc::fence_after_sync();
           if (tc::elect_one()) {
@@ -364,7 +379,7 @@
               tc::mma_ss<false>(tmem_d, t_hi, d_hi, Cfg::kIdesc, 1u);
             }
             tc::mma_commit(&t_empty[ts]);
-            if (part == XW_PARTS - 1) {
+            if (part == parts - 1) {
               tc::mma_commit(&d_empty[ds]);
               if (kb == KB - 1) tc::mma_commit(&tfull[buf]);
             }
@@ -380,16 +395,18 @@
     const int quad = warp & 3;
     int it = 0;
     for (int cell = blockIdx.x; cell < cells.n_cells; cell += gridDim.x) {
-      if (box_org[cell].y == INT_MIN) continue;
+      const XwBox bx = box[cell];
+      if (bx.parts == 0) continue;
       const int m = cells.m[cell], map0 = cells.row0[cell];
+      const int part_tok = (bx.width == XW_BOX ? XW_ROWS_WIDE : XW_ROWS_NARROW) * bx.width;
       const int buf = it % Cfg::kAccBufs, use = it / Cfg::kAccBufs;
       tc::mbar_wait(&tfull[buf], use & 1);
       tc::fence_after_sync();
       const int tok = quad * 32 + lane;
 #pragma unroll 1
-      for (int part = 0; part < XW_PARTS; ++part) {
-        const int col = part * XW_PART_TOK + tok;
-        const bool ok = tok < XW_PART_TOK && col < XW_BOX * XW_BOX;
+      for (int part = 0; part < bx.parts; ++part) {
+        const int col = part * part_tok + tok;
+        const bool ok = tok < part_tok && col < bx.height * bx.width;
         const uint32_t taddr = tmem_base + ((uint32_t)(quad * 32) << 16) + buf * Cfg::kAccCols + part * NB;
         float* dst = xbox + (size_t)map0 * XW_COLS + col;
 #pragma unroll 1
@@ -425,18 +442,17 @@
   DTK_CHECK_ARG(fv.C % 8 == 0 && cells.max_m <= XW_MAX_CELL, "exact-window GEMM: bad sizes");
   const bool small = cells.max_m <= 64;
   const int nb = small ? 64 : 128;
-  CUtensorMap tD_hi, tD_lo, tT_hi, tT_lo, tL_hi, tL_lo;
+  CUtensorMap tD_hi, tD_lo, tN_hi, tN_lo, tW_hi, tW_lo;
   int rc;
   if ((rc = make_tmap_2d(&tD_hi, desc_hi, desc_rows, fv.C, nb, 64, TMAP_F16))) return rc;
   if ((rc = make_tmap_2d(&tD_lo, desc_lo, desc_rows, fv.C, nb, 64, TMAP_F16))) return rc;
   const uint64_t dims[4] = {(uint64_t)fv.C, (uint64_t)g.w, (uint64_t)g.h, (uint64_t)fv.T};
   const uint64_t strides[3] = {(uint64_t)fv.C * 2, (uint64_t)g.w * fv.C * 2, (uint64_t)fv.P * fv.C * 2};
-  const uint32_t box[4] = {64, XW_BOX, XW_PART_ROWS, 1};
-  if ((rc = make_tmap_4d(&tT_hi, fv.hi, dims, strides, box, TMAP_F16))) return rc;
-  if ((rc = make_tmap_4d(&tT_lo, fv.lo, dims, strides, box, TMAP_F16))) return rc;
-  const uint32_t box_last[4] = {64, XW_BOX, (uint32_t)XwCfg<64>::kLastRows, 1};
-  if ((rc = make_tmap_4d(&tL_hi, fv.hi, dims, strides, box_last, TMAP_F16))) return rc;
-  if ((rc = make_tmap_4d(&tL_lo, fv.lo, dims, strides, box_last, TMAP_F16))) return rc;
+  const uint32_t box_n[4] = {64, XW_NARROW, XW_ROWS_NARROW, 1}, box_w[4] = {64, XW_BOX, XW_ROWS_WIDE, 1};
+  if ((rc = make_tmap_4d(&tN_hi, fv.hi, dims, strides, box_n, TMAP_F16))) return rc;
+  if ((rc = make_tmap_4d(&tN_lo, fv.lo, dims, strides, box_n, TMAP_F16))) return rc;
+  if ((rc = make_tmap_4d(&tW_hi, fv.hi, dims, strides, box_w, TMAP_F16))) return rc;
+  if ((rc = make_tmap_4d(&tW_lo, fv.lo, dims, strides, box_w, TMAP_F16))) return rc;
   static PerDev<bool> attr_dev;
   bool& attr = attr_dev.get();
   if (!attr) {
@@ -450,9 +466,9 @@
   const int grid = cells.n_cells < sms ? cells.n_cells : sms;
   ProfRange pr(PROF_XW_GEMM, st);
   if (small)
-    xw_gemm_kernel<64><<<grid, TC_THREADS, XwCfg<64>::kSmem, st>>>(tD_hi, tD_lo, tT_hi, tT_lo, tL_hi, tL_lo, cells, xc.box_org, xc.xbox, fv.C);
+    xw_gemm_kernel<64><<<grid, TC_THREADS, XwCfg<64>::kSmem, st>>>(tD_hi, tD_lo, tN_hi, tN_lo, tW_hi, tW_lo, cells, xc.box, xc.xbox, fv.C);
   else
-    xw_gemm_kernel<128><<<grid, TC_THREADS, XwCfg<128>::kSmem, st>>>(tD_hi, tD_lo, tT_hi, tT_lo, tL_hi, tL_lo, cells, xc.box_org, xc.xbox, fv.C);
+    xw_gemm_kernel<128><<<grid, TC_THREADS, XwCfg<128>::kSmem, st>>>(tD_hi, tD_lo, tN_hi, tN_lo, tW_hi, tW_lo, cells, xc.box, xc.xbox, fv.C);
   DTK_LAUNCHED();
   return DINOTRK_OK;
 }
@@ -597,7 +613,7 @@
 constexpr int XWIN_PITCH = 256;
 __global__ void __launch_bounds__(256)
 xw_window_kernel(int n_maps, int h, int w, int P, int n_tiles, const float* __restrict__ norms, const float* __restrict__ desc_norm,
-                 const int* __restrict__ cell_frame, const int* __restrict__ cell_of, const int2* __restrict__ box_org,
+                 const int* __restrict__ cell_frame, const int* __restrict__ cell_of, const XwBox* __restrict__ box,
                  const int* __restrict__ stat, const int* __restrict__ cand, const unsigned long long* __restrict__ key1,
                  const float* __restrict__ max2, const float* __restrict__ xbox, float* __restrict__ win, int2* __restrict__ hin) {
   const int lane = threadIdx.x & 31;
@@ -608,7 +624,7 @@
       continue;
     }
     const int cell = cell_of[map];
-    const int2 org = box_org[cell];
+    const XwBox bx = box[cell];
     const float* fn = norms + (size_t)cell_frame[cell] * P;
     const float* xr = xbox + (size_t)map * XW_COLS;
     const float dn = desc_norm[map];
@@ -620,7 +636,7 @@
     for (int q = 0; q < XW_MAX_CAND; ++q)
       if (ct[q] >= 0) {
         const int tr = ct[q] / w, tcn = ct[q] - tr * w;
-        const float v = fmaxf(__fdiv_rn(__ldg(xr + xw_col(tr - org.x, tcn - org.y)), fmaxf(__fmul_rn(dn, __ldg(fn + ct[q])), 1e-8f)), 0.f);
+        const float v = fmaxf(__fdiv_rn(__ldg(xr + xw_col(tr - bx.row, tcn - bx.col, bx.width)), fmaxf(__fmul_rn(dn, __ldg(fn + ct[q])), 1e-8f)), 0.f);
         if (v > best || (v == best && ct[q] < amax)) { best = v; amax = ct[q]; }
       }
     const int arow = amax / w, acol = amax - arow * w;
@@ -640,7 +656,7 @@
       const int r = arow - 7 + y, c = acol - 7 + x;
       float v = 0.f;
       if (y < XWM && x < XWM && r >= 0 && r < h && c >= 0 && c < w) {
-        v = fmaxf(__fdiv_rn(__ldg(xr + xw_col(r - org.x, c - org.y)), fmaxf(__fmul_rn(dn, __ldg(fn + r * w + c)), 1e-8f)), 0.f);
+        v = fmaxf(__fdiv_rn(__ldg(xr + xw_col(r - bx.row, c - bx.col, bx.width)), fmaxf(__fmul_rn(dn, __ldg(fn + r * w + c)), 1e-8f)), 0.f);
         if (!(abs(r - arow) <= 3 && abs(c - acol) <= 3)) mout = fmaxf(mout, v);
       }
       win[(size_t)map * XWIN_PITCH + i] = v;
@@ -763,7 +779,7 @@
   {
     int wgrid = cdiv(n_maps, 8);
     if (wgrid > sms * 8) wgrid = sms * 8;
-    xw_window_kernel<<<wgrid, 256, 0, st>>>(n_maps, g.h, g.w, hp.P, hp.n_tiles, fv.norms, desc_norm, cells.frame, xc.cell_of, xc.box_org,
+    xw_window_kernel<<<wgrid, 256, 0, st>>>(n_maps, g.h, g.w, hp.P, hp.n_tiles, fv.norms, desc_norm, cells.frame, xc.cell_of, xc.box,
                                             xc.stat, xc.cand, xc.key1, xc.max2, xc.xbox, xc.win, xc.hin);
     DTK_LAUNCHED();
   }
@@ -829,10 +845,10 @@
   size_t b = 0;
   b += align_up(ch * n_tiles * 8, 256) + align_up(ch * n_tiles * 4, 256);
   b += align_up(ch * XW_MAX_CAND * 4, 256) + 4 * align_up(ch * 4, 256);
-  b += align_up((size_t)max_cells * 8, 256);
+  b += align_up((size_t)max_cells * sizeof(XwBox), 256);
   b += align_up(ch * XW_COLS * 4, 256);
   b += align_up(ch * 256 * 4, 256) + align_up(ch * 8, 256);
-  b += align_up((size_t)(gcap + 2) * 4, 256);
+  b += align_up((size_t)(gcap + XW_NCNT) * 4, 256);
   return b + 2048;
 }
 
diff --git a/dino_tracker_b200/csrc/xwin.cuh b/dino_tracker_b200/csrc/xwin.cuh
--- a/dino_tracker_b200/csrc/xwin.cuh
+++ b/dino_tracker_b200/csrc/xwin.cuh
@@ -7,15 +7,22 @@
 constexpr float XW_EPS = 1.1e-3f;
 constexpr int XW_BOX = 21;
 constexpr int XW_SLACK = 3;
-constexpr int XW_PARTS = 4, XW_PART_ROWS = 6;
-constexpr int XW_PART_TOK = XW_PART_ROWS * XW_BOX;
+constexpr int XW_NARROW = 16;
+constexpr int XW_ROWS_NARROW = 8, XW_ROWS_WIDE = 6;
+constexpr int XW_PARTS = 4;
 constexpr int XW_COLS = 448;
 constexpr int XW_MAX_CELL = 128;
 constexpr int XW_MAX_CAND = 4;
 constexpr float XW_MIN_NORM = 1e-4f;
 constexpr int XW_TILE = 128;
+constexpr int XW_NCNT = 2 + (XW_PARTS - 1);
 
-__host__ __device__ inline int xw_col(int by, int bx) { return by * XW_BOX + bx; }
+__host__ __device__ inline int xw_col(int by, int bx, int width) { return by * width + bx; }
+
+struct __align__(16) XwBox {
+  int row, col;
+  short width, height, parts;
+};
 
 struct XwChunk {
   unsigned long long* key1;
@@ -24,7 +31,7 @@
   int* pinfo;
   int* stat;
   int* cell_of;
-  int2* box_org;
+  XwBox* box;
   float* xbox;
   float* win;
   int2* hin;
```
